# JakobHavtorn/benchmarking-lvms

Hardware: AMD Instinct MI355X
Metric: audio frames/sec training (VRNN, 16 kHz mu-law) (higher is better)
Workload: dtype f32

## Files before the change

benchmarking-lvms_amd/csrc/pchain.h:

```cpp
#pragma once
#include <algorithm>
#include <cstdlib>

#include "common.h"

namespace blvm {
namespace pchain {

constexpr unsigned SENTINEL = 0xFFFFFFFFu;
constexpr unsigned SPIN_LIMIT = 1u << 22;

typedef unsigned u32x4 __attribute__((ext_vector_type(4)));
typedef __amdgpu_buffer_rsrc_t rsrc_t;
constexpr int AUX_SC1 = 16;
#ifndef PCHAIN_POLL_AUX
#define PCHAIN_POLL_AUX AUX_SC1
#endif
#ifndef PCHAIN_STORE_AUX
#define PCHAIN_STORE_AUX AUX_SC1
#endif
__device__ __forceinline__ rsrc_t make_rsrc(const void* base) {
  const unsigned long long u = reinterpret_cast<unsigned long long>(base);
  const unsigned lo = (unsigned)__builtin_amdgcn_readfirstlane((int)(unsigned)u), hi = (unsigned)__builtin_amdgcn_readfirstlane((int)(unsigned)(u >> 32));
  return __builtin_amdgcn_make_buffer_rsrc(reinterpret_cast<void*>(((unsigned long long)hi << 32) | lo), 0, 0xFFFFFFFFu, 0x00020000);
}
__device__ __forceinline__ f32x4 ld_sc1_x4(rsrc_t r, unsigned byte_off) {
  return __builtin_bit_cast(f32x4, __builtin_amdgcn_raw_buffer_load_b128(r, (int)byte_off, 0, PCHAIN_POLL_AUX));
}
__device__ __forceinline__ float ld_sc1(rsrc_t r, unsigned byte_off) {
  return __builtin_bit_cast(float, __builtin_amdgcn_raw_buffer_load_b32(r, (int)byte_off, 0, PCHAIN_POLL_AUX));
}
__device__ __forceinline__ void st_sc1(rsrc_t r, unsigned byte_off, float v) {
  __builtin_amdgcn_raw_buffer_store_b32(__builtin_bit_cast(unsigned, v), r, (int)byte_off, 0, PCHAIN_STORE_AUX);
}

__device__ __forceinline__ bool is_sentinel(float x) { return __float_as_uint(x) == SENTINEL; }
__device__ __forceinline__ bool any_sentinel(const f32x4& v) {
  return is_sentinel(v[0]) | is_sentinel(v[1]) | is_sentinel(v[2]) | is_sentinel(v[3]);
}

struct Ctl {
  unsigned* dev;
  unsigned* host;
  unsigned epoch;
  __device__ __forceinline__ bool aborted() const { return __hip_atomic_load(dev, __ATOMIC_RELAXED, __HIP_MEMORY_SCOPE_AGENT) == epoch; }
  __device__ __forceinline__ void abort(unsigned code) const {
    if (__hip_atomic_exchange(dev, epoch, __ATOMIC_RELAXED, __HIP_MEMORY_SCOPE_AGENT) != epoch) {
      __hip_atomic_store(host + 1, code, __ATOMIC_RELAXED, __HIP_MEMORY_SCOPE_SYSTEM);
      __hip_atomic_fetch_add(host, 1u, __ATOMIC_RELAXED, __HIP_MEMORY_SCOPE_SYSTEM);
    }
  }
};

__device__ __forceinline__ bool spin_tick(unsigned& spins, const Ctl& ctl, unsigned code, bool& dead) {
  ++spins;
  if ((spins & 255u) == 0) {
    if (ctl.aborted()) { dead = true; return true; }
    if (spins >= SPIN_LIMIT) { ctl.abort(code); dead = true; return true; }
  }
  return false;
}

struct Poll {
  Ctl ctl;
  unsigned code;
  bool dead;
  int nap;
#ifdef PCHAIN_TPROF
  unsigned long long t_first = 0, t_ok = 0, t_end = 0, tp[8] = {0, 0, 0, 0, 0, 0, 0, 0};
  unsigned polls = 0;
#endif
  __device__ __forceinline__ void sleep() const {
    if (nap > 8) __builtin_amdgcn_s_sleep(32);
    else __builtin_amdgcn_s_sleep(1);
  }
};

struct MapSame { static constexpr int of(int) { return 0; } static constexpr bool sum = false; };
struct MapId { static constexpr int of(int g) { return g; } static constexpr bool sum = false; };
struct MapPairs { static constexpr int of(int g) { return g >> 1; } static constexpr bool sum = false; };
struct MapSum { static constexpr int of(int) { return 0; } static constexpr bool sum = true; };

struct NoMid {
  __device__ __forceinline__ void operator()() const {}
};

typedef short s16x4 __attribute__((ext_vector_type(4)));
typedef unsigned u32x2 __attribute__((ext_vector_type(2)));
typedef float f32x2_t __attribute__((ext_vector_type(2)));
typedef __bf16 bf16x2_t __attribute__((ext_vector_type(2)));
typedef _Float16 f16x2_t __attribute__((ext_vector_type(2)));
typedef _Float16 f16x4_t __attribute__((ext_vector_type(4)));
__device__ __forceinline__ unsigned pk_bf16(float a, float b) {
  return __builtin_bit_cast(unsigned, __builtin_convertvector((f32x2_t){a, b}, bf16x2_t));
}
template <int OT>
__device__ __forceinline__ unsigned pk16(float a, float b) {
  if constexpr (OT == OP_F16) return __builtin_bit_cast(unsigned, __builtin_convertvector((f32x2_t){a, b}, f16x2_t));
  else return pk_bf16(a, b);
}
template <int OT>
__device__ __forceinline__ f32x4 mfma16(s16x4 a, s16x4 b, f32x4 acc) {
  if constexpr (OT == OP_F16)
    return __builtin_amdgcn_mfma_f32_16x16x16f16(__builtin_bit_cast(f16x4_t, a), __builtin_bit_cast(f16x4_t, b), acc, 0, 0, 0);
  else return __builtin_amdgcn_mfma_f32_16x16x16bf16_1k(a, b, acc, 0, 0, 0);
}
template <int OT> struct WFrag { typedef u32x2 type; };
template <> struct WFrag<OP_F32> { typedef f32x4 type; };

template <int NW, int OT, int GA, int G, class AMap, int CH, class Mid>
__device__ __forceinline__ void mgemm_trip(const rsrc_t (&ar)[GA], unsigned aoff, const float* const (&ap)[GA], const char* const (&wp)[G], int kc,
                                           bool aok, bool polled, f32x4 (&acc)[G], Poll& pl, Mid& mid, bool& mid_pending) {
  constexpr int STEP = NW * 16;
  typedef typename WFrag<OT>::type wfrag;
  constexpr int ES = OT != OP_F32 ? 2 : 4;
  wfrag w[G][CH];
  f32x4 a[GA][CH];
#pragma unroll
  for (int u = 0; u < CH; ++u)
#pragma unroll
    for (int g = 0; g < G; ++g) w[g][u] = *reinterpret_cast<const wfrag*>(wp[g] + (size_t)ES * 16 * (size_t)(kc + u * STEP));
  if (!polled) {
#pragma unroll
    for (int u = 0; u < CH; ++u)
#pragma unroll
      for (int g = 0; g < GA; ++g) a[g][u] = *reinterpret_cast<const f32x4*>(ap[g] + kc + u * STEP);
    if (mid_pending) { mid(); mid_pending = false; }
  } else {
    unsigned spins = 0;
    for (;;) {
#pragma unroll
      for (int u = 0; u < CH; ++u)
#pragma unroll
        for (int g = 0; g < GA; ++g) a[g][u] = ld_sc1_x4(ar[g], aoff + 64u * (unsigned)(kc + u * STEP));
      if (mid_pending) { mid(); mid_pending = false; }
      bool bad = false;
#pragma unroll
      for (int u = 0; u < CH; ++u)
#pragma unroll
        for (int g = 0; g < GA; ++g) bad |= any_sentinel(a[g][u]);
#ifdef PCHAIN_TPROF
      if (spins == 0 && pl.t_first == 0) pl.t_first = wall_clock64();
      pl.polls++;
#endif
      if (!__any(bad && aok) || pl.dead) break;
      if (spin_tick(spins, pl.ctl, pl.code, pl.dead)) break;
      pl.sleep();
    }
#ifdef PCHAIN_TPROF
    pl.t_ok = wall_clock64();
#endif
  }
  if constexpr (AMap::sum) {
#pragma unroll
    for (int u = 0; u < CH; ++u)
#pragma unroll
      for (int ga = 1; ga < GA; ++ga) a[0][u] += a[ga][u];
  }
  if constexpr (OT != OP_F32) {
#pragma unroll
    for (int u = 0; u < CH; ++u) {
      s16x4 ab[GA];
#pragma unroll
      for (int ga = 0; ga < GA; ++ga) {
        const f32x4 x = a[ga][u];
        const u32x2 q = {aok ? pk16<OT>(x[0], x[1]) : 0u, aok ? pk16<OT>(x[2], x[3]) : 0u};
        ab[ga] = __builtin_bit_cast(s16x4, q);
      }
#pragma unroll
      for (int g = 0; g < G; ++g) acc[g] = mfma16<OT>(ab[AMap::of(g)], __builtin_bit_cast(s16x4, w[g][u]), acc[g]);
    }
  } else {
#pragma unroll
    for (int u = 0; u < CH; ++u)
#pragma unroll
      for (int e = 0; e < 4; ++e)
#pragma unroll
        for (int g = 0; g < G; ++g) acc[g] = __builtin_amdgcn_mfma_f32_16x16x4f32(aok ? a[AMap::of(g)][u][e] : 0.f, w[g][u][e], acc[g], 0, 0, 0);
  }
}

template <int NW, int OT, int GA, int G, class AMap, class Mid = NoMid>
__device__ __forceinline__ void mgemm16(const float* const (&A)[GA], const int (&lda)[GA], bool polled, int r0, int nrows,
                                        const float* const (&W)[G], const int (&c0)[G], int K, f32x4 (&acc)[G], Poll& pl, Mid mid = Mid(),
                                        int a_width = 0, int w_width = 0) {
  constexpr int STEP = NW * 16;
  constexpr int FR = (NW >= 16 ? 6 : 12) / (G + GA);
  constexpr int MAXCH = FR >= 6 ? 6 : (FR >= 4 ? 4 : (FR >= 2 ? 2 : 1));
  const int lane = threadIdx.x & 63, wave = threadIdx.x >> 6;
  const int rr = lane & 15, q = lane >> 4;
  const bool aok = (r0 + rr) < nrows;
  rsrc_t ar[GA];
  const float* ap[GA];
  const char* wp[G];
#pragma unroll
  for (int g = 0; g < GA; ++g) {
    ar[g] = make_rsrc(A[g]);
    ap[g] = A[g] + (size_t)(aok ? r0 + rr : r0) * (polled ? 0 : lda[g]) + 4 * q;
  }
  const unsigned aoff = 4u * ((unsigned)(r0 >> 4) * 16u * (unsigned)(a_width > 0 ? a_width : K) + 4u * (unsigned)lane);
#pragma unroll
  for (int g = 0; g < G; ++g) wp[g] = reinterpret_cast<const char*>(W[g]) + (OT != OP_F32 ? 2 : 4) * ((size_t)c0[g] * (w_width > 0 ? w_width : K) + 4 * lane);
  int nch = (K / 16 - wave + NW - 1) / NW;
  int kc = wave * 16;
  bool mid_pending = true;
  if constexpr (MAXCH >= 6) for (; nch >= 6; nch -= 6, kc += 6 * STEP) mgemm_trip<NW, OT, GA, G, AMap, 6>(ar, aoff, ap, wp, kc, aok, polled, acc, pl, mid, mid_pending);
  if constexpr (MAXCH >= 4) for (; nch >= 4; nch -= 4, kc += 4 * STEP) mgemm_trip<NW, OT, GA, G, AMap, 4>(ar, aoff, ap, wp, kc, aok, polled, acc, pl, mid, mid_pending);
  if constexpr (MAXCH >= 2) for (; nch >= 2; nch -= 2, kc += 2 * STEP) mgemm_trip<NW, OT, GA, G, AMap, 2>(ar, aoff, ap, wp, kc, aok, polled, acc, pl, mid, mid_pending);
  for (; nch >= 1; nch -= 1, kc += STEP) mgemm_trip<NW, OT, GA, G, AMap, 1>(ar, aoff, ap, wp, kc, aok, polled, acc, pl, mid, mid_pending);
  if (mid_pending) mid();
}

template <int N>
__device__ __forceinline__ void poll_words(const rsrc_t (&r)[N], const unsigned (&off)[N], float (&v)[N], bool need, Poll& pl) {
  unsigned spins = 0;
  for (;;) {
#pragma unroll
    for (int i = 0; i < N; ++i) v[i] = ld_sc1(r[i], off[i]);
    bool bad = false;
#pragma unroll
    for (int i = 0; i < N; ++i) bad |= is_sentinel(v[i]);
    if (!__any(bad && need) || pl.dead) break;
    if (spin_tick(spins, pl.ctl, pl.code, pl.dead)) break;
    pl.sleep();
  }
}

__device__ __forceinline__ int first_tile(int w, int wg0, int nwg, int ntiles) {
  return (w >= wg0 && w < wg0 + nwg) ? w - wg0 : ntiles;
}

struct TileIter {
  int rt, ct, j, step, x, n;
  bool xcd;
  __host__ __device__ __forceinline__ TileIter(int w, int wg0, int nwg, int rt_, int ct_, bool xcd_) : rt(rt_), ct(ct_), xcd(xcd_) {
    const int wl = w - wg0;
    const bool in = w >= wg0 && wl < nwg;
    if (xcd) {
      x = wl & 7; step = nwg >> 3; j = wl >> 3;
      n = x < ct ? ((ct - x + 7) >> 3) * rt : 0;
    } else {
      x = 0; step = nwg; j = wl;
      n = rt * ct;
    }
    if (!in || step < 1) { j = 0; n = 0; step = 1; x = 0; }
  }
  __host__ __device__ __forceinline__ bool valid() const { return j < n; }
  __host__ __device__ __forceinline__ void next() { j += step; }
  __host__ __device__ __forceinline__ int r0() const { return (j % rt) * 16; }
  __host__ __device__ __forceinline__ int c() const { return xcd ? x + 8 * (j / rt) : j / rt; }
};

inline int tiles_per_workgroup(int rt, int ct, int nwg, bool xcd) {
  if (nwg <= 0) return 0;
  if (xcd) return nwg >= 8 ? (((ct + 7) / 8) * rt + nwg / 8 - 1) / (nwg / 8) : ((ct + 7) / 8) * rt;
  return (ct * rt + nwg - 1) / nwg;
}

__device__ __forceinline__ void canary_wait(const float* A16, int r0, int K, Poll& pl, int a_width = 0) {
  if (threadIdx.x < 64) {
    const int lane = threadIdx.x, np = K >> 4;
    const rsrc_t r = make_rsrc(A16 + (size_t)(r0 >> 4) * 16 * (a_width > 0 ? a_width : K));
    unsigned spins = 0;
    for (;;) {
      bool bad = false;
      for (int p0 = 0; p0 < np; p0 += 64) {
        const int pr = p0 + lane;
        const float v = ld_sc1(r, 1024u * (unsigned)(pr < np ? pr : 0));
        bad |= (pr < np) && is_sentinel(v);
      }
      if (!__any(bad) || pl.dead) break;
      if (spin_tick(spins, pl.ctl, pl.code, pl.dead)) break;
      pl.sleep();
    }
  }
  __syncthreads();
}

struct WMem {
  static constexpr bool resident = false;
  static constexpr int products = 0;
};
template <int OT, int G, int NCH>
struct WRegs {
  static constexpr bool resident = true;
  static constexpr int products = G;
  typename WFrag<OT>::type w[G][NCH];
};
template <int NW, int OT, int G, int NCH>
__device__ __forceinline__ void load_w(typename WFrag<OT>::type (&w)[G][NCH], const float* const* W, const int (&c0)[G], int ldw) {
  typedef typename WFrag<OT>::type wfrag;
  const int lane = threadIdx.x & 63, wave = threadIdx.x >> 6;
  constexpr int ES = OT != OP_F32 ? 2 : 4;
#pragma unroll
  for (int g = 0; g < G; ++g) {
    const char* base = reinterpret_cast<const char*>(W[g]) + (size_t)ES * ((size_t)c0[g] * ldw + 4 * lane);
#pragma unroll
    for (int u = 0; u < NCH; ++u) w[g][u] = *reinterpret_cast<const wfrag*>(base + (size_t)ES * 256 * (size_t)(wave + u * NW));
  }
}
template <int NW, int OT, int GA, int G, class AMap, int NCH, bool SHARED, class Mid>
__device__ __forceinline__ void product_regs(const float* const (&A16)[GA], int r0, int nrows, int width,
                                             const typename WFrag<OT>::type (&w)[G][NCH], f32x4 (&acc)[G], Poll& pl, Mid mid) {
  static_assert(!SHARED || GA == 1, "the shared-slab form reads one operand");
  const int lane = threadIdx.x & 63, wave = threadIdx.x >> 6;
  const bool aok = (r0 + (lane & 15)) < nrows;
  rsrc_t ar[GA];
#pragma unroll
  for (int g = 0; g < GA; ++g) ar[g] = make_rsrc(A16[g]);
  const unsigned aoff = 4u * ((unsigned)(r0 >> 4) * 16u * (unsigned)width + 4u * (unsigned)lane) + 1024u * (unsigned)wave;
  f32x4 a[GA][NCH];
  unsigned spins = 0;
  bool mid_pending = true;
  if constexpr (SHARED) {
    canary_wait(A16[0], r0, width, pl);
    const float* ap = A16[0] + (size_t)(r0 >> 4) * 16 * width + 4 * lane + 256 * wave;
#pragma unroll
    for (int u = 0; u < NCH; ++u) a[0][u] = *reinterpret_cast<const f32x4*>(ap + 256 * (size_t)(u * NW));
    mid();
    mid_pending = false;
    bool bad = false;
#pragma unroll
    for (int u = 0; u < NCH; ++u) bad |= any_sentinel(a[0][u]);
    if (!__any(bad && aok)) goto multiply;
  }
  for (;;) {
#pragma unroll
    for (int u = 0; u < NCH; ++u)
#pragma unroll
      for (int g = 0; g < GA; ++g) a[g][u] = ld_sc1_x4(ar[g], aoff + 1024u * (unsigned)(u * NW));
    if (mid_pending) { mid(); mid_pending = false; }
    bool bad = false;
#pragma unroll
    for (int u = 0; u < NCH; ++u)
#pragma unroll
      for (int g = 0; g < GA; ++g) bad |= any_sentinel(a[g][u]);
    if (!__any(bad && aok) || pl.dead) break;
    if (spin_tick(spins, pl.ctl, pl.code, pl.dead)) break;
    pl.sleep();
  }
multiply:
  if constexpr (AMap::sum) {
#pragma unroll
    for (int u = 0; u < NCH; ++u)
#pragma unroll
      for (int ga = 1; ga < GA; ++ga) a[0][u] += a[ga][u];
  }
  if constexpr (OT != OP_F32) {
#pragma unroll
    for (int u = 0; u < NCH; ++u) {
      s16x4 ab[GA];
#pragma unroll
      for (int ga = 0; ga < GA; ++ga) {
        const f32x4 x = a[ga][u];
        const u32x2 q = {aok ? pk16<OT>(x[0], x[1]) : 0u, aok ? pk16<OT>(x[2], x[3]) : 0u};
        ab[ga] = __builtin_bit_cast(s16x4, q);
      }
#pragma unroll
      for (int g = 0; g < G; ++g) acc[g] = mfma16<OT>(ab[AMap::of(g)], __builtin_bit_cast(s16x4, w[g][u]), acc[g]);
    }
  } else {
#pragma unroll
    for (int u = 0; u < NCH; ++u)
#pragma unroll
      for (int e = 0; e < 4; ++e)
#pragma unroll
        for (int g = 0; g < G; ++g) acc[g] = __builtin_amdgcn_mfma_f32_16x16x4f32(aok ? a[AMap::of(g)][u][e] : 0.f, w[g][u][e], acc[g], 0, 0, 0);
  }
}

template <int NW, int OT, int GA, int G, class AMap, class Mid = NoMid>
__device__ __forceinline__ void tile_product(const WMem&, const float* const (&A)[GA], const int (&lda)[GA], bool polled, int r0, int nrows,
                                             const float* const (&W)[G], const int (&c0)[G], int K, f32x4 (&acc)[G], Poll& pl, Mid mid = Mid(),
                                             int a_width = 0, int w_width = 0) {
  mgemm16<NW, OT, GA, G, AMap>(A, lda, polled, r0, nrows, W, c0, K, acc, pl, mid, a_width, w_width);
}
template <int NW, int OT, int GA, int G, class AMap, class Mid = NoMid, int NCH>
__device__ __forceinline__ void tile_product(const WRegs<OT, G, NCH>& ws, const float* const (&A)[GA], const int (&)[GA], bool, int r0, int nrows,
                                             const float* const (&)[G], const int (&)[G], int, f32x4 (&acc)[G], Poll& pl, Mid mid = Mid(),
                                             int a_width = 0, int = 0) {
  product_regs<NW, OT, GA, G, AMap, NCH, false>(A, r0, nrows, a_width > 0 ? a_width : NCH * 16 * NW, ws.w, acc, pl, mid);
}

struct Out {
  float* rm;
  int ld;
  bool rm_sc1;
  float* x16;
  int n16;
  float* x16b = nullptr;
  int n16b = 0;
};
__device__ __forceinline__ Out out_rm(float* p, int ld, bool sc1 = false) { return Out{p, ld, sc1, nullptr, 0}; }
__device__ __forceinline__ Out out_both(float* p, int ld, float* x16, int n16, bool sc1 = false) { return Out{p, ld, sc1, x16, n16}; }
__device__ __forceinline__ void put(const Out& o, int r0, int c0, int row, int col, float x) {
  if (o.rm != nullptr) {
    if (o.rm_sc1) st_sc1(make_rsrc(o.rm), 4u * ((unsigned)row * (unsigned)o.ld + (unsigned)col), x);
    else o.rm[(size_t)row * o.ld + col] = x;
  }
  const int rr = row - r0, cc = col - c0;
  const unsigned in_block = (unsigned)((rr + 16 * ((cc & 15) >> 2)) * 4 + (cc & 3));
  if (o.x16 != nullptr) st_sc1(make_rsrc(o.x16), 4u * ((((unsigned)(r0 >> 4) * (unsigned)o.n16 + (unsigned)((c0 + cc) >> 4)) << 8) + in_block), x);
  if (o.x16b != nullptr) st_sc1(make_rsrc(o.x16b), 4u * ((((unsigned)(r0 >> 4) * (unsigned)o.n16b + (unsigned)((c0 + cc) >> 4)) << 8) + in_block), x);
}


struct LinLate {
  const float *bias, *add, *gate;
  int ldadd, ldgate;
  bool add_polled, relu;
  float slope;
  Out out;
};
template <int NW, int OT, class Late, class WS = WMem>
__device__ __forceinline__ void tile_lin_late(const float* A, int lda, bool a_polled, const float* W, int K, Late& late, int r0, int c0, int B,
                                              float* red, Poll& pl, const float* A2 = nullptr, const float* A3 = nullptr, int w_width = 0,
                                              const WS& ws = WS()) {
  const int t = threadIdx.x & 255;
  const int row = r0 + (t >> 4), col = c0 + (t & 15);
  const bool own = threadIdx.x < 256 && row < B;
  const int rowc = row < B ? row : r0;
#ifdef PCHAIN_TPROF
  const unsigned long long t0 = wall_clock64();
  pl.t_first = 0; pl.polls = 0;
#endif
  float e_bias = 0.f, e_gate = 1.f, e_add = 0.f;
  LinLate L;
  auto prefetch = [&]() {
    L = late();
    if (L.bias) e_bias = L.bias[col];
    if (L.gate) e_gate = L.gate[(size_t)rowc * L.ldgate + col];
    if (L.add && !L.add_polled) e_add = L.add[(size_t)rowc * L.ldadd + col];
  };
  f32x4 acc[1] = {{0.f, 0.f, 0.f, 0.f}};
  if (A2 != nullptr) {
    const float* const As[3] = {A, A2, A3};
    const float* const Ws[1] = {W};
    const int la[3] = {0, 0, 0}, cs[1] = {c0};
    tile_product<NW, OT, 3, 1, MapSum>(ws, As, la, true, r0, B, Ws, cs, K, acc, pl, prefetch, lda, w_width);
  } else {
    const float* const As[1] = {A};
    const float* const Ws[1] = {W};
    const int la[1] = {lda}, cs[1] = {c0};
    tile_product<NW, OT, 1, 1, MapSame>(ws, As, la, a_polled, r0, B, Ws, cs, K, acc, pl, prefetch, a_polled ? lda : 0, w_width);
  }
  float v[1];
  reduce_tiles<1, NW>(acc, red, v);
#ifdef PCHAIN_TPROF
  if (a_polled && pl.nap == 1) {
    const unsigned long long t3 = wall_clock64();
    pl.tp[0] += 1; pl.tp[1] += pl.t_first - t0; pl.tp[2] += pl.t_ok - pl.t_first; pl.tp[3] += t3 - pl.t_ok; pl.tp[4] += pl.polls;
    if (pl.t_end != 0) pl.tp[6] += t0 - pl.t_end;
  }
#endif
  if (threadIdx.x >= 256) return;
  if (L.add && L.add_polled) {
    const rsrc_t rs[1] = {make_rsrc(L.add)};
    const unsigned os[1] = {4u * ((unsigned)rowc * (unsigned)L.ldadd + (unsigned)col)};
    float ws[1];
    poll_words<1>(rs, os, ws, own, pl);
    e_add = ws[0];
  }
  if (!own) return;
  float x = v[0] + e_bias + e_add;
  if (L.relu) x = x > 0.f ? x : x * L.slope;
  if (L.gate) x = e_gate > 0.f ? x : x * L.slope;
  put(L.out, r0, c0, row, col, x);
#ifdef PCHAIN_TPROF
  if (a_polled && pl.nap == 1) { pl.t_end = wall_clock64(); }
#endif
}
template <int NW, int OT = OP_F32>
__device__ __forceinline__ void tile_lin(const float* A, int lda, bool a_polled, const float* W, int K, const float* bias,
                                         const float* add, int ldadd, bool add_polled, const float* gate, int ldgate, bool relu,
                                         float slope, const Out& out, int r0, int c0, int B, float* red, Poll& pl) {
  auto late = [&]() { return LinLate{bias, add, gate, ldadd, ldgate, add_polled, relu, slope, out}; };
  tile_lin_late<NW, OT>(A, lda, a_polled, W, K, late, r0, c0, B, red, pl);
}

struct HeadOut {
  float *mu_p, *sd_p, *mu_q, *sd_q, *raw_p, *raw_q, *muq_raw;
  Out z;
};
template <int NW, int OT = OP_F32, class WS = WMem>
__device__ __forceinline__ void tile_head(const float* P, const float* Q, bool polled, const float* Wp, const float* bp, const float* Wq,
                                          const float* bq, const float* eps, const HeadOut& o, int H, int Z, int residual, float beta,
                                          float inv_beta, float sd_eps, int r0, int c0, int B, float* red, Poll& pl, const WS& ws = WS()) {
  const int t = threadIdx.x & 255;
  const int row = r0 + (t >> 4), col = c0 + (t & 15);
  const bool own = threadIdx.x < 256 && row < B;
  const size_t oc = (size_t)(row < B ? row : r0) * Z + col;
  float b0 = 0.f, b1 = 0.f, b2 = 0.f, b3 = 0.f, e = 0.f;
  auto prefetch = [&]() { b0 = bp[col]; b1 = bp[Z + col]; b2 = bq[col]; b3 = bq[Z + col]; e = eps[oc]; };
  f32x4 acc[4];
#pragma unroll
  for (int g = 0; g < 4; ++g) acc[g] = (f32x4){0.f, 0.f, 0.f, 0.f};
  {
    const float* const As[2] = {P, Q};
    const float* const Ws[4] = {Wp, Wp, Wq, Wq};
    const int la[2] = {H, H}, cs[4] = {c0, Z + c0, c0, Z + c0};
    tile_product<NW, OT, 2, 4, MapPairs>(ws, As, la, polled, r0, B, Ws, cs, H, acc, pl, prefetch);
  }
  float v[4];
  reduce_tiles<4, NW>(acc, red, v);
  if (!own) return;
  const size_t oo = (size_t)row * Z + col;
  const float mp = v[0] + b0, rp = v[1] + b1, rq = v[3] + b3;
  float mq = v[2] + b2;
  const float sp = softplus_beta(rp, beta, inv_beta) + sd_eps;
  const float sq = softplus_beta(rq, beta, inv_beta) + sd_eps;
  if (o.muq_raw != nullptr) o.muq_raw[oo] = mq;
  float sqc = sq;
  if (residual == 1) {
    mq += mp;
  } else if (residual == 2) {
    const float pq = 1.f / (sq * sq), pp = 1.f / (sp * sp);
    const float var = 1.f / (pq + pp);
    mq = var * (mq * pq + mp * pp);
    sqc = sqrtf(var);
  } else if (residual == 3) {
    mq = mp;
    sqc = sp;
  }
  put(o.z, r0, c0, row, col, e * sqc + mq);
  o.mu_p[oo] = mp; o.sd_p[oo] = sp; o.mu_q[oo] = mq; o.sd_q[oo] = sqc;
  o.raw_p[oo] = rp; o.raw_q[oo] = rq;
}

template <int NW, int OT = OP_F32, class WS = WMem>
__device__ __forceinline__ void tile_gru(const float* X, int ldx, bool polled, const float* Wih, int K, const float* xg, const float* bih,
                                         const float* gh, const float* hprev, int ldh, int R, const Out& hnew, float* rg, float* ug, float* ng,
                                         int r0, int c0, int B, float* red, Poll& pl, const WS& ws = WS()) {
  const int t = threadIdx.x & 255;
  const int row = r0 + (t >> 4), col = c0 + (t & 15);
  const bool own = threadIdx.x < 256 && row < B;
  const int rowc = row < B ? row : r0;
  const size_t o3 = (size_t)rowc * 3 * R + col;
  const rsrc_t rgh = make_rsrc(gh), rhp = make_rsrc(hprev);
  const rsrc_t ps[4] = {rgh, rgh, rgh, rhp};
  const unsigned po[4] = {4u * (unsigned)o3, 4u * (unsigned)(o3 + R), 4u * (unsigned)(o3 + 2 * R), 4u * ((unsigned)rowc * (unsigned)ldh + (unsigned)col)};
  float w[4] = {0.f, 0.f, 0.f, 0.f}, x0 = 0.f, x1 = 0.f, x2 = 0.f;
  auto prefetch = [&]() {
#pragma unroll
    for (int i = 0; i < 4; ++i) w[i] = ld_sc1(ps[i], po[i]);
    x0 = (xg ? xg[o3] : 0.f) + (bih ? bih[col] : 0.f);
    x1 = (xg ? xg[o3 + R] : 0.f) + (bih ? bih[R + col] : 0.f);
    x2 = (xg ? xg[o3 + 2 * R] : 0.f) + (bih ? bih[2 * R + col] : 0.f);
  };
  f32x4 acc[3];
#pragma unroll
  for (int g = 0; g < 3; ++g) acc[g] = (f32x4){0.f, 0.f, 0.f, 0.f};
  {
    const float* const As[1] = {X};
    const float* const Ws[3] = {Wih, Wih, Wih};
    const int la[1] = {ldx}, cs[3] = {c0, R + c0, 2 * R + c0};
    tile_product<NW, OT, 1, 3, MapSame>(ws, As, la, polled, r0, B, Ws, cs, K, acc, pl, prefetch);
  }
  float v[3];
  reduce_tiles<3, NW>(acc, red, v);
  if (threadIdx.x >= 256) return;
  if (__any(own && (is_sentinel(w[0]) | is_sentinel(w[1]) | is_sentinel(w[2]) | is_sentinel(w[3])))) poll_words<4>(ps, po, w, own, pl);
  if (!own) return;
  const float r = sigmoidf_(v[0] + x0 + w[0]);
  const float u = sigmoidf_(v[1] + x1 + w[1]);
  const float n = tanhf(v[2] + x2 + r * w[2]);
  put(hnew, r0, c0, row, col, (1.f - u) * n + u * w[3]);
  const size_t o = (size_t)row * R + col;
  rg[o] = r; ug[o] = u; ng[o] = n;
}

struct DzIn {
  const float *mu_q, *sd_q, *mu_p, *sd_p, *eps, *raw_q, *raw_p, *muq_raw;
  const int32_t* x_sl;
  const float *c_raw, *c_fn;
  int t, stride, residual;
  float fn_floor, beta, sd_eps;
  bool has_gemm = true;
};
template <int NW, int OT = OP_F32, class WS = WMem>
__device__ __forceinline__ void tile_dz(const float* D, const float* WT, const float* D2, const float* WT2, bool polled, const float* dz_add,
                                        int ld_add, bool add_polled, const DzIn& a, const Out& dqh, const Out& dph, int H, int Z, int r0, int c0,
                                        int B, float* red, Poll& pl, const WS& ws = WS()) {
  const int t = threadIdx.x & 255;
  const int row = r0 + (t >> 4), col = c0 + (t & 15);
  const bool own = threadIdx.x < 256 && row < B;
  const int rowc = row < B ? row : r0;
  const size_t o = (size_t)rowc * Z + col;
  float mq = 0.f, sq = 1.f, mp = 0.f, sp = 1.f, e = 0.f, rq = 0.f, rp = 0.f, c_raw = 0.f, c_fn = 0.f, e_add = 0.f;
  auto prefetch = [&]() {
    mq = a.mu_q[o]; sq = a.sd_q[o]; mp = a.mu_p[o]; sp = a.sd_p[o]; e = a.eps[o]; rq = a.raw_q[o]; rp = a.raw_p[o];
    if (a.c_fn != nullptr || a.c_raw != nullptr) {
      const bool live = (long long)a.t * a.stride < a.x_sl[rowc];
      c_raw = (live && a.c_raw != nullptr) ? a.c_raw[rowc] : 0.f;
      c_fn = (live && a.c_fn != nullptr) ? a.c_fn[rowc] : 0.f;
    }
    if (dz_add != nullptr && !add_polled) e_add = dz_add[(size_t)rowc * ld_add + col];
  };
  float v[2] = {0.f, 0.f};
  if (a.has_gemm) {
    f32x4 acc[2];
    acc[0] = (f32x4){0.f, 0.f, 0.f, 0.f};
    acc[1] = (f32x4){0.f, 0.f, 0.f, 0.f};
    if (WS::products != 1 && D2 != nullptr) {
      if constexpr (WS::products != 1) {
        const float* const As[2] = {D, D2};
        const float* const Ws[2] = {WT, WT2};
        const int la[2] = {H, H}, cs[2] = {c0, c0};
        tile_product<NW, OT, 2, 2, MapId>(ws, As, la, polled, r0, B, Ws, cs, H, acc, pl, prefetch);
      }
    } else {
      if constexpr (WS::products != 2) {
        f32x4 a1[1] = {acc[0]};
        const float* const As[1] = {D};
        const float* const Ws[1] = {WT};
        const int la[1] = {H}, cs[1] = {c0};
        tile_product<NW, OT, 1, 1, MapSame>(ws, As, la, polled, r0, B, Ws, cs, H, a1, pl, prefetch);
        acc[0] = a1[0];
      }
    }
    reduce_tiles<2, NW>(acc, red, v);
  } else {
    prefetch();
  }
  if (threadIdx.x >= 256) return;
  if (dz_add != nullptr && add_polled) {
    const rsrc_t rs[1] = {make_rsrc(dz_add)};
    const unsigned os[1] = {4u * ((unsigned)rowc * (unsigned)ld_add + (unsigned)col)};
    float ws[1];
    poll_words<1>(rs, os, ws, own, pl);
    e_add = ws[0];
  }
  if (!own) return;
  const float dz = v[0] + v[1] + e_add;
  const float d = mq - mp, ip2 = 1.f / (sp * sp);
  float coef = c_raw;
  if (c_fn != 0.f) {
    const float k = logf(sp) - logf(sq) + (sq * sq + d * d) * 0.5f * ip2 - 0.5f;
    if (!(a.fn_floor > 0.f) || k > a.fn_floor) coef += c_fn;
  }
  float g_muq = dz + coef * d * ip2;
  float g_sdq = dz * e + coef * (sq * ip2 - 1.f / sq);
  float g_mup = -coef * d * ip2;
  float g_sdp = coef * (1.f / sp - (sq * sq + d * d) * ip2 / sp);
  if (a.residual == 1) {
    g_mup += g_muq;
  } else if (a.residual == 2) {
    const float mqr = a.muq_raw[o];
    const float sqr = softplus_beta(rq, a.beta, 1.f / a.beta) + a.sd_eps;
    const float pq = 1.f / (sqr * sqr), pp = ip2, var = sq * sq;
    const float half_s3 = 0.5f * var * sq;
    const float g_pq = g_muq * var * (mqr - mq) - g_sdq * half_s3;
    const float g_pp = g_muq * var * (mp - mq) - g_sdq * half_s3;
    g_mup += g_muq * var * pp;
    g_sdp += g_pp * (-2.f * pp / sp);
    g_sdq = g_pq * (-2.f * pq / sqr);
    g_muq = g_muq * var * pq;
  }
  put(dqh, r0, c0, row, col, g_muq);
  put(dqh, r0, Z + c0, row, Z + col, g_sdq * sigmoidf_(a.beta * rq));
  put(dph, r0, c0, row, col, g_mup);
  put(dph, r0, Z + c0, row, Z + col, g_sdp * sigmoidf_(a.beta * rp));
}

struct GrubIn {
  const float *D0, *D1, *W0, *W1, *g_in, *g_add;
  const float *rg, *ug, *ng, *gh, *hprev, *dd;
  int ldh, ld_gadd;
  Out dgi, dgh;
  float *ga, *g_out;
  bool has_gemm, has_gin, has_gates;
};
template <int NW, int OT = OP_F32, class WS = WMem>
__device__ __forceinline__ void tile_grub(const GrubIn& a, int K, int R, int r0, int c0, int B, float* red, Poll& pl, const WS& ws = WS()) {
  const int tt = threadIdx.x & 255;
  const int row = r0 + (tt >> 4), col = c0 + (tt & 15);
  const bool own = threadIdx.x < 256 && row < B;
  const int rowc = row < B ? row : r0;
  const size_t o = (size_t)rowc * R + col, o3 = (size_t)rowc * 3 * R + col;
  float r = 0.f, u = 0.f, n = 0.f, hn = 0.f, hp = 0.f, dd = 0.f, gadd = 0.f, g0 = 0.f;
  auto prefetch = [&]() {
    if (a.has_gin) g0 = ld_sc1(make_rsrc(a.g_in), 4u * (unsigned)o);
    if (a.has_gates) {
      r = a.rg[o]; u = a.ug[o]; n = a.ng[o]; hn = a.gh[o3 + 2 * R];
      hp = a.hprev[(size_t)rowc * a.ldh + col];
      if (a.dd != nullptr) dd = a.dd[(size_t)rowc * a.ldh + col];
    }
    if (a.g_add != nullptr) gadd = a.g_add[(size_t)rowc * a.ld_gadd + col];
  };
  float v[2] = {0.f, 0.f};
  if (!a.has_gemm) prefetch();
  if (a.has_gemm) {
    f32x4 acc[2];
    acc[0] = (f32x4){0.f, 0.f, 0.f, 0.f};
    acc[1] = (f32x4){0.f, 0.f, 0.f, 0.f};
    const float* const As[2] = {a.D0, a.D1};
    const float* const Ws[2] = {a.W0, a.W1};
    const int la[2] = {0, 0}, cs[2] = {c0, c0};
    tile_product<NW, OT, 2, 2, MapId>(ws, As, la, true, r0, B, Ws, cs, K, acc, pl, prefetch);
    reduce_tiles<2, NW>(acc, red, v);
  }
  if (threadIdx.x >= 256) return;
  if (a.has_gin && __any(own && is_sentinel(g0))) {
    const rsrc_t rs[1] = {make_rsrc(a.g_in)};
    const unsigned os[1] = {4u * (unsigned)o};
    float ws[1];
    poll_words<1>(rs, os, ws, own, pl);
    g0 = ws[0];
  }
  if (!own) return;
  const float g = (g0 + gadd) + v[0] + v[1];
  if (!a.has_gates) { a.g_out[(size_t)row * R + col] = g; return; }
  const float dn_pre = g * (1.f - u) * (1.f - n * n);
  const float du_pre = g * (hp - n) * u * (1.f - u);
  const float dr_pre = dn_pre * hn * r * (1.f - r);
  put(a.dgi, r0, c0, row, col, dr_pre); put(a.dgi, r0, R + c0, row, R + col, du_pre); put(a.dgi, r0, 2 * R + c0, row, 2 * R + col, dn_pre);
  put(a.dgh, r0, c0, row, col, dr_pre); put(a.dgh, r0, R + c0, row, R + col, du_pre); put(a.dgh, r0, 2 * R + c0, row, 2 * R + col, dn_pre * r);
  st_sc1(make_rsrc(a.ga), 4u * ((unsigned)row * (unsigned)R + (unsigned)col), g * u + dd);
}

__device__ __forceinline__ int seq_time_index(int j, int reverse, const int32_t* lens, int row) {
  if (!reverse) return j;
  const int n = lens[row];
  return j < n ? n - 1 - j : j;
}
struct GruSeqIn {
  const float *H16, *Whh, *bhh;
  const float* xg;
  const int32_t* lens;
  const float* hprev;
  float* out;
  float *rg, *ug, *ng, *ghn;
  long out_ts;
  int out_ld, j, reverse;
};
template <int NW, int OT = OP_F32>
__device__ __forceinline__ void tile_gru_seq(const GruSeqIn& a, const Out& hnext, int R, int r0, int c0, int B, float* red, Poll& pl) {
  const int t = threadIdx.x & 255;
  const int row = r0 + (t >> 4), col = c0 + (t & 15);
  const bool own = threadIdx.x < 256 && row < B;
  const int rowc = row < B ? row : r0;
  const size_t o = (size_t)rowc * R + col;
  int idx = 0;
  float x0 = 0.f, x1 = 0.f, x2 = 0.f, b0 = 0.f, b1 = 0.f, b2 = 0.f, hp = 0.f;
  auto prefetch = [&]() {
    idx = seq_time_index(a.j, a.reverse, a.lens, rowc);
    const size_t ox = ((size_t)idx * B + rowc) * 3 * R + col;
    x0 = a.xg[ox]; x1 = a.xg[ox + R]; x2 = a.xg[ox + 2 * R];
    b0 = a.bhh[col]; b1 = a.bhh[R + col]; b2 = a.bhh[2 * R + col];
    hp = a.hprev[o];
  };
  f32x4 acc[3];
#pragma unroll
  for (int g = 0; g < 3; ++g) acc[g] = (f32x4){0.f, 0.f, 0.f, 0.f};
  {
    const float* const As[1] = {a.H16};
    const float* const Ws[3] = {a.Whh, a.Whh, a.Whh};
    const int la[1] = {0}, cs[3] = {c0, R + c0, 2 * R + c0};
    mgemm16<NW, OT, 1, 3, MapSame>(As, la, true, r0, B, Ws, cs, R, acc, pl, prefetch);
  }
  float v[3];
  reduce_tiles<3, NW>(acc, red, v);
  if (!own) return;
  const float hn = v[2] + b2;
  const float r = sigmoidf_(x0 + v[0] + b0);
  const float u = sigmoidf_(x1 + v[1] + b1);
  const float n = tanhf(x2 + r * hn);
  const float h2 = (1.f - u) * n + u * hp;
  put(hnext, r0, c0, row, col, h2);
  a.out[(size_t)idx * a.out_ts + (size_t)row * a.out_ld + col] = h2;
  a.rg[o] = r; a.ug[o] = u; a.ng[o] = n; a.ghn[o] = hn;
}

struct GruSeqBwdIn {
  const float *DGHn16, *WhhT;
  const float* dout;
  const float *rg, *ug, *ng, *ghn, *hprev;
  const int32_t* lens;
  float* G;
  float* DGI;
  float* dh0;
  long out_ts;
  int out_ld, j, reverse;
  bool has_gemm, has_gates;
};
template <int NW, int OT = OP_F32>
__device__ __forceinline__ void tile_gru_seq_bwd(const GruSeqBwdIn& a, const Out& dgh, int R, int r0, int c0, int B, float* red, Poll& pl) {
  const int t = threadIdx.x & 255;
  const int row = r0 + (t >> 4), col = c0 + (t & 15);
  const bool own = threadIdx.x < 256 && row < B;
  const int rowc = row < B ? row : r0;
  const size_t o = (size_t)rowc * R + col;
  float g = 0.f, dout = 0.f, r = 0.f, u = 0.f, n = 0.f, hn = 0.f, hp = 0.f;
  int idx = 0;
  auto prefetch = [&]() {
    g = a.G[o];
    if (a.has_gates) {
      idx = seq_time_index(a.j, a.reverse, a.lens, rowc);
      dout = a.dout[(size_t)idx * a.out_ts + (size_t)rowc * a.out_ld + col];
      r = a.rg[o]; u = a.ug[o]; n = a.ng[o]; hn = a.ghn[o]; hp = a.hprev[o];
    }
  };
  float v[1] = {0.f};
  if (a.has_gemm) {
    f32x4 acc[1] = {{0.f, 0.f, 0.f, 0.f}};
    const float* const As[1] = {a.DGHn16};
    const float* const Ws[1] = {a.WhhT};
    const int la[1] = {0}, cs[1] = {c0};
    mgemm16<NW, OT, 1, 1, MapSame>(As, la, true, r0, B, Ws, cs, 3 * R, acc, pl, prefetch);
    reduce_tiles<1, NW>(acc, red, v);
  } else {
    prefetch();
    __syncthreads();
  }
  if (!own) return;
  g += dout + v[0];
  if (!a.has_gates) { a.dh0[o] = g; return; }
  const float dn_pre = g * (1.f - u) * (1.f - n * n);
  const float du_pre = g * (hp - n) * u * (1.f - u);
  const float dr_pre = dn_pre * hn * r * (1.f - r);
  const size_t oi = ((size_t)idx * B + row) * 3 * R + col;
  a.DGI[oi] = dr_pre; a.DGI[oi + R] = du_pre; a.DGI[oi + 2 * R] = dn_pre;
  put(dgh, r0, c0, row, col, dr_pre);
  put(dgh, r0, R + c0, row, R + col, du_pre);
  put(dgh, r0, 2 * R + c0, row, 2 * R + col, dn_pre * r);
  a.G[o] = g * u;
}

struct LstmSeqIn {
  const float *H16, *Whh, *bhh;
  const float* xg;
  const int32_t* lens;
  const float *hprev, *cprev;
  float *cnext, *out, *gates;
  int t;
};
template <int NW, int OT = OP_F32>
__device__ __forceinline__ void tile_lstm_seq(const LstmSeqIn& a, const Out& hnext, int H, int r0, int c0, int B, float* red, Poll& pl) {
  const int tt = threadIdx.x & 255;
  const int row = r0 + (tt >> 4), col = c0 + (tt & 15);
  const bool own = threadIdx.x < 256 && row < B;
  const int rowc = row < B ? row : r0;
  const size_t o = (size_t)rowc * H + col, o4 = (size_t)rowc * 4 * H + col;
  float x0 = 0.f, x1 = 0.f, x2 = 0.f, x3 = 0.f, hp = 0.f, cp = 0.f;
  bool live = true;
  auto prefetch = [&]() {
    x0 = a.xg[o4] + a.bhh[col]; x1 = a.xg[o4 + H] + a.bhh[H + col];
    x2 = a.xg[o4 + 2 * H] + a.bhh[2 * H + col]; x3 = a.xg[o4 + 3 * H] + a.bhh[3 * H + col];
    hp = a.hprev[o]; cp = a.cprev[o];
    live = a.lens == nullptr || a.t < a.lens[rowc];
  };
  f32x4 acc[4];
#pragma unroll
  for (int g = 0; g < 4; ++g) acc[g] = (f32x4){0.f, 0.f, 0.f, 0.f};
  {
    const float* const As[1] = {a.H16};
    const float* const Ws[4] = {a.Whh, a.Whh, a.Whh, a.Whh};
    const int la[1] = {0}, cs[4] = {c0, H + c0, 2 * H + c0, 3 * H + c0};
    mgemm16<NW, OT, 1, 4, MapSame>(As, la, true, r0, B, Ws, cs, H, acc, pl, prefetch);
  }
  float v[4];
  reduce_tiles<4, NW>(acc, red, v);
  if (!own) return;
  const float i = sigmoidf_(v[0] + x0), f = sigmoidf_(v[1] + x1), g = tanhf(v[2] + x2), og = sigmoidf_(v[3] + x3);
  const float c2 = f * cp + i * g;
  const float h2 = og * tanhf(c2);
  a.cnext[o] = live ? c2 : cp;
  put(hnext, r0, c0, row, col, live ? h2 : hp);
  a.out[o] = live ? h2 : 0.f;
  a.gates[o4] = live ? i : 0.f;
  a.gates[o4 + H] = live ? f : 0.f;
  a.gates[o4 + 2 * H] = live ? g : 0.f;
  a.gates[o4 + 3 * H] = live ? og : 0.f;
}

struct LstmSeqBwdIn {
  const float *DGn16, *WhhT;
  const float *dout, *gates, *c_s, *c_s1;
  float* DC;
  float* dh0;
  bool has_gemm, has_gates;
};
template <int NW, int OT = OP_F32>
__device__ __forceinline__ void tile_lstm_seq_bwd(const LstmSeqBwdIn& a, const Out& dg, int H, int r0, int c0, int B, float* red, Poll& pl) {
  const int tt = threadIdx.x & 255;
  const int row = r0 + (tt >> 4), col = c0 + (tt & 15);
  const bool own = threadIdx.x < 256 && row < B;
  const int rowc = row < B ? row : r0;
  const size_t o = (size_t)rowc * H + col, o4 = (size_t)rowc * 4 * H + col;
  float dh = 0.f, ig = 0.f, fg = 0.f, gg = 0.f, og = 0.f, cs = 0.f, cs1 = 0.f, dc = 0.f;
  auto prefetch = [&]() {
    if (a.has_gates) {
      dh = a.dout[o];
      ig = a.gates[o4]; fg = a.gates[o4 + H]; gg = a.gates[o4 + 2 * H]; og = a.gates[o4 + 3 * H];
      cs = a.c_s[o]; cs1 = a.c_s1[o]; dc = a.DC[o];
    }
  };
  float v[1] = {0.f};
  if (a.has_gemm) {
    f32x4 acc[1] = {{0.f, 0.f, 0.f, 0.f}};
    const float* const As[1] = {a.DGn16};
    const float* const Ws[1] = {a.WhhT};
    const int la[1] = {0}, cs_[1] = {c0};
    mgemm16<NW, OT, 1, 1, MapSame>(As, la, true, r0, B, Ws, cs_, 4 * H, acc, pl, prefetch);
    reduce_tiles<1, NW>(acc, red, v);
  } else {
    prefetch();
    __syncthreads();
  }
  if (!own) return;
  dh += v[0];
  if (!a.has_gates) { a.dh0[o] = dh; return; }
  const float tc = tanhf(cs1);
  const float d_o = dh * tc;
  const float dct = dc + dh * og * (1.f - tc * tc);
  put(dg, r0, c0, row, col, dct * gg * ig * (1.f - ig));
  put(dg, r0, H + c0, row, H + col, dct * cs * fg * (1.f - fg));
  put(dg, r0, 2 * H + c0, row, 2 * H + col, dct * ig * (1.f - gg * gg));
  put(dg, r0, 3 * H + c0, row, 3 * H + col, d_o * og * (1.f - og));
  a.DC[o] = dct * fg;
}

template <int NW, int OT = OP_F32>
__device__ __forceinline__ void tile_lstm(const float* X, const float* Wih, int K, const float* bih, const float* gh, const float* cprev, float* cnext, int H,
                                          const Out& hnew, int r0, int c0, int B, float* red, Poll& pl) {
  const int t = threadIdx.x & 255;
  const int row = r0 + (t >> 4), col = c0 + (t & 15);
  const bool own = threadIdx.x < 256 && row < B;
  const int rowc = row < B ? row : r0;
  const size_t o = (size_t)rowc * H + col, o4 = (size_t)rowc * 4 * H + col;
  const rsrc_t rgh = make_rsrc(gh);
  const rsrc_t ps[4] = {rgh, rgh, rgh, rgh};
  const unsigned po[4] = {4u * (unsigned)o4, 4u * (unsigned)(o4 + H), 4u * (unsigned)(o4 + 2 * H), 4u * (unsigned)(o4 + 3 * H)};
  float w[4] = {0.f, 0.f, 0.f, 0.f}, b0 = 0.f, b1 = 0.f, b2 = 0.f, b3 = 0.f, cp = 0.f;
  auto prefetch = [&]() {
#pragma unroll
    for (int i = 0; i < 4; ++i) w[i] = ld_sc1(ps[i], po[i]);
    b0 = bih[col]; b1 = bih[H + col]; b2 = bih[2 * H + col]; b3 = bih[3 * H + col];
    cp = cprev[o];
  };
  f32x4 acc[4];
#pragma unroll
  for (int g = 0; g < 4; ++g) acc[g] = (f32x4){0.f, 0.f, 0.f, 0.f};
  {
    const float* const As[1] = {X};
    const float* const Ws[4] = {Wih, Wih, Wih, Wih};
    const int la[1] = {0}, cs[4] = {c0, H + c0, 2 * H + c0, 3 * H + c0};
    mgemm16<NW, OT, 1, 4, MapSame>(As, la, true, r0, B, Ws, cs, K, acc, pl, prefetch);
  }
  float v[4];
  reduce_tiles<4, NW>(acc, red, v);
  if (threadIdx.x >= 256) return;
  if (__any(own && (is_sentinel(w[0]) | is_sentinel(w[1]) | is_sentinel(w[2]) | is_sentinel(w[3])))) poll_words<4>(ps, po, w, own, pl);
  if (!own) return;
  const float i = sigmoidf_(v[0] + b0 + w[0]), f = sigmoidf_(v[1] + b1 + w[1]), g = tanhf(v[2] + b2 + w[2]), og = sigmoidf_(v[3] + b3 + w[3]);
  const float c2 = f * cp + i * g;
  cnext[(size_t)row * H + col] = c2;
  put(hnew, r0, c0, row, col, og * tanhf(c2));
}

template <int NW>
__device__ __forceinline__ void tile_dmol_sample(const float* dec, int ldd, const float* Wl, const float* bl, const float* u, const float* v, int S, int F,
                                                 int num_mix, float log_eps, const Out& xo, int r0, int s0, int B, float* lds, Poll& pl) {
  static_assert(NW == 8 || NW == 16, "waves");
  const int tid = threadIdx.x, wave = tid >> 6, lane = tid & 63;
  float* in = lds;
  float* outp = lds + 16 * 4 * F;
  const int rowlen = 4 * F;
  const int pieces = 16 * rowlen / 4;
  const rsrc_t rd = make_rsrc(dec);
  {
    unsigned spins = 0;
    for (;;) {
      bool bad = false;
      for (int q = tid; q < pieces; q += NW * 64) {
        const int rr = q / (rowlen / 4), cq = q % (rowlen / 4);
        const bool ok = r0 + rr < B;
        const f32x4 x = ld_sc1_x4(rd, 4u * ((unsigned)(ok ? r0 + rr : r0) * (unsigned)ldd + (unsigned)(s0 * F + 4 * cq)));
        bad |= ok && any_sentinel(x);
        *reinterpret_cast<f32x4*>(in + rr * rowlen + 4 * cq) = x;
      }
      if (!__any(bad) || pl.dead) break;
      if (spin_tick(spins, pl.ctl, pl.code, pl.dead)) break;
      pl.sleep();
    }
  }
  __syncthreads();
  {
    const int rr = lane >> 2, ss = lane & 3;
    const float* a = in + rr * rowlen + ss * F;
    if (wave * 4 < F) {
      float acc[4];
#pragma unroll
      for (int j = 0; j < 4; ++j) {
        const int jj = wave * 4 + j;
        acc[j] = jj < F ? bl[jj] : 0.f;
      }
      for (int k = 0; k < F; ++k) {
        const float ak = a[k];
#pragma unroll
        for (int j = 0; j < 4; ++j) {
          const int jj = wave * 4 + j;
          if (jj < F) acc[j] = fmaf(Wl[jj * F + k], ak, acc[j]);
        }
      }
#pragma unroll
      for (int j = 0; j < 4; ++j)
        if (wave * 4 + j < F) outp[lane * 32 + wave * 4 + j] = acc[j];
    }
  }
  __syncthreads();
  if (wave == 0) {
    const int rr = lane >> 2, ss = lane & 3, row = r0 + rr, smp = s0 + ss;
    if (row < B) {
      const float* p = outp + lane * 32;
      const size_t f = (size_t)row * S + smp;
      int best = 0;
      float bv = -INFINITY;
      for (int m = 0; m < num_mix; ++m) {
        float sc = p[m];
        if (u != nullptr) sc -= logf(-logf(u[f * num_mix + m]));
        if (sc > bv) { bv = sc; best = m; }
      }
      const float loc = p[num_mix + best], raw = p[2 * num_mix + best];
      float x = loc;
      if (v != nullptr) {
        const float vv = v[f];
        x = loc + expf(fmaxf(raw, log_eps)) * (logf(vv) - logf(1.f - vv));
        x = fminf(fmaxf(x, -1.f), 1.f);
      }
      put(xo, r0, s0 & ~15, row, smp, x);
    }
  }
  __syncthreads();
}

enum Kind : int { K_LIN = 0, K_HEAD = 1, K_GRU = 2, K_DZ = 3, K_GRUB = 4, K_DMOLS = 5, K_GRUS = 6, K_GRUSB = 7, K_LSTMS = 8, K_LSTMSB = 9, K_LINSEQ = 10, K_LSTM = 11 };
enum DescFlag : int {
  DF_RELU = 1,
  DF_A_PLAIN = 2,
  DF_ADD_POLLED = 4,
  DF_RM_SC1 = 8,
  DF_GENTLE = 16,
  DF_CANARY = 32,
  DF_A_SUM3 = 64,
  DF_SEQ_GATE = 128,
};
enum : int { LD_OUT = 3, N16_OUT = 0, N16_OUTB = 1 };
enum : int { LIN_A, LIN_W, LIN_BIAS, LIN_ADD, LIN_GATE, LIN_ORM, LIN_O16, LIN_O16B, LIN_A2, LIN_A3, LIN_LD_A = 0, LIN_LD_ADD = 1, LIN_LD_GATE = 2,
             LIN_I_W_WIDTH = 0, LIN_F_SLOPE = 0 };
enum : int { LINSEQ_A0 = 0, LINSEQ_W = 1, LINSEQ_AUX = 5, LINSEQ_ORM = 9, LINSEQ_O16 = 13, LINSEQ_ADD0 = 17, LINSEQ_LD_ORM = 0,
             LINSEQ_I_LD_ADD0 = 0, LINSEQ_I_N = 1, LINSEQ_I_LD_GATE = 2, LINSEQ_I_K0 = 3, LINSEQ_F_SLOPE = 0 };
enum : int { HEAD_P16, HEAD_Q16, HEAD_WP, HEAD_BP, HEAD_WQ, HEAD_BQ, HEAD_EPS, HEAD_MU_P, HEAD_SD_P, HEAD_MU_Q, HEAD_SD_Q, HEAD_RAW_P, HEAD_RAW_Q,
             HEAD_MUQ_RAW, HEAD_Z, HEAD_Z16, HEAD_Z16B, HEAD_I_Z = 0, HEAD_I_RESIDUAL = 1, HEAD_F_BETA = 0, HEAD_F_INV_BETA = 1, HEAD_F_SD_EPS = 2 };
enum : int { GRU_X16, GRU_WIH, GRU_XG, GRU_GH, GRU_HPREV, GRU_HRM, GRU_H16, GRU_RG, GRU_UG, GRU_NG, GRU_BIH, GRU_H16B, GRU_LD_HPREV = 0, GRU_I_R = 0 };
enum : int { DZ_D16, DZ_WT, DZ_D2_16, DZ_WT2, DZ_ADD, DZ_MU_Q, DZ_SD_Q, DZ_MU_P, DZ_SD_P, DZ_EPS, DZ_RAW_Q, DZ_RAW_P, DZ_MUQ_RAW, DZ_X_SL, DZ_C_RAW,
             DZ_C_FN, DZ_DQH, DZ_DQH16, DZ_DPH, DZ_DPH16, DZ_LD_ADD = 1, DZ_I_Z = 0, DZ_I_RESIDUAL = 1, DZ_I_STRIDE = 2, DZ_I_T0 = 3,
             DZ_F_FN_FLOOR = 0, DZ_F_BETA = 1, DZ_F_SD_EPS = 2, DZ_F_GEMM_FROM = 3 };
enum : int { GRUB_D0_16, GRUB_D1_16, GRUB_W0, GRUB_W1, GRUB_G_IN, GRUB_RG, GRUB_UG, GRUB_NG, GRUB_GH, GRUB_HPREV, GRUB_DD, GRUB_DGI, GRUB_DGI16,
             GRUB_DGH, GRUB_DGH16, GRUB_GA, GRUB_G_OUT, GRUB_G_ADD, GRUB_LD_H = 0, GRUB_LD_GADD = 1, GRUB_I_R = 0, GRUB_I_GEMM_FROM = 1,
             GRUB_I_GATES_TO = 2, GRUB_I_GIN_FROM = 3 };
enum : int { DMOLS_DEC, DMOLS_W, DMOLS_B, DMOLS_U, DMOLS_V, DMOLS_X, DMOLS_X16, DMOLS_LD_DEC = 0, DMOLS_I_S = 0, DMOLS_I_F = 1, DMOLS_I_NMIX = 2,
             DMOLS_F_LOG_EPS = 0 };
enum : int { GRUS_H16, GRUS_WHH, GRUS_BHH, GRUS_XG, GRUS_LENS, GRUS_HPREV, GRUS_HNEXT, GRUS_HNEXT16, GRUS_OUT, GRUS_RG, GRUS_UG, GRUS_NG, GRUS_GHN,
             GRUS_I_R = 0, GRUS_I_REVERSE = 1, GRUS_I_OUT_TS = 2, GRUS_I_OUT_LD = 3 };
enum : int { GRUSB_DGH16_IN, GRUSB_WHHT, GRUSB_DOUT, GRUSB_RG, GRUSB_UG, GRUSB_NG, GRUSB_GHN, GRUSB_HPREV, GRUSB_LENS, GRUSB_G, GRUSB_DGI, GRUSB_DGH,
             GRUSB_DGH16, GRUSB_DH0, GRUSB_N16_T = 1, GRUSB_I_R = 0, GRUSB_I_REVERSE = 1, GRUSB_I_OUT_TS = 2, GRUSB_I_OUT_LD = 3 };
enum : int { LSTMS_H16, LSTMS_WHH, LSTMS_BHH, LSTMS_XG, LSTMS_LENS, LSTMS_HPREV, LSTMS_HNEXT, LSTMS_HNEXT16, LSTMS_CPREV, LSTMS_CNEXT, LSTMS_OUT,
             LSTMS_GATES, LSTMS_I_H = 0 };
enum : int { LSTMSB_DG16_IN, LSTMSB_WHHT, LSTMSB_DOUT, LSTMSB_GATES, LSTMSB_CS, LSTMSB_DC, LSTMSB_DG, LSTMSB_DG16, LSTMSB_DH0, LSTMSB_N16_T = 1, LSTMSB_I_H = 0 };
enum : int { LSTM_X16, LSTM_WIH, LSTM_BIH, LSTM_GH, LSTM_CPREV, LSTM_CNEXT, LSTM_HRM, LSTM_H16, LSTM_H16B, LSTM_I_H = 0 };
constexpr int kMaxDesc = 24, kMaxPtr = 20;
struct Desc {
  int kind, ct, wg0, nwg, flags, K, s_begin, s_end;
  int ld[4];
  int n16[2];
  int i[4];
  float f[4];
  unsigned char sidx[kMaxPtr];
  const float* p[kMaxPtr];
};
struct Program {
  int ot = OP_F32;
  int rt_group = 1;
  int s_first = 0;
  int ndesc, S, B, xcd;
  long stride[16];
  Ctl ctl;
  unsigned long long* prof;
  int prof_wg, lds_products;
  Desc d[kMaxDesc];
};

struct Ptr {
  const void* p; long step;
  Ptr(const void* p_ = nullptr, long step_ = 0) : p(p_), step(step_) {}
};
struct Builder {
  Program p{};
  int nstride = 1;
  bool overflow = false;
  void begin(int ot, int S, int B, int lds_products, bool backward, int prof_wg) {
    p.ot = ot; p.S = S; p.B = B; p.xcd = (pchain_tune() & 4) ? 1 : 0; p.lds_products = lds_products;
    p.prof = pchain_profile_buffer() && backward ? pchain_profile_buffer() + 64 : pchain_profile_buffer(); p.prof_wg = prof_wg;
  }
  int stride_index(long v) {
    if (v == 0) return 0;
    for (int i = 1; i < nstride; ++i)
      if (p.stride[i] == v) return i;
    if (nstride >= 16) { overflow = true; return 0; }
    p.stride[nstride] = v;
    return nstride++;
  }
  Desc& add(int kind, int ct, int wg0, int nwg, int K, int flags, int s_begin, int s_end) {
    static Desc dummy;
    if (p.ndesc >= kMaxDesc) { overflow = true; return dummy; }
    Desc& d = p.d[p.ndesc++];
    d = Desc{};
    d.kind = kind; d.ct = ct; d.wg0 = wg0; d.nwg = nwg; d.K = K; d.flags = flags; d.s_begin = s_begin; d.s_end = s_end;
    return d;
  }
  void ptr(Desc& d, int k, Ptr q) {
    d.p[k] = static_cast<const float*>(q.p);
    d.sidx[k] = (unsigned char)(q.p ? stride_index(q.step) : 0);
  }
};
inline Ptr rev(const float* base, long step, long t0) { return Ptr(base ? base + t0 * step : nullptr, -step); }

struct Operands {
  Ptr p[kMaxPtr];
  int ld[4] = {}, n16[2] = {}, i[4] = {}; float f[4] = {};
};
inline Desc& add_desc(Builder& b, int kind, int ct, int wg0, int nwg, int K, int flags, int s_begin, int s_end, const Operands& o) {
  Desc& d = b.add(kind, ct, wg0, nwg, K, flags, s_begin, s_end);
  for (int k = 0; k < kMaxPtr; ++k) b.ptr(d, k, o.p[k]);
  std::copy(o.ld, o.ld + 4, d.ld); std::copy(o.n16, o.n16 + 2, d.n16); std::copy(o.i, o.i + 4, d.i); std::copy(o.f, o.f + 4, d.f);
  return d;
}

struct SeqLink {
  const float *W, *aux;
  float* orm;
  long rm_step;
  int ldo;
  float* o16;
};
inline Desc& add_linseq(Builder& b, int ct, int wg0, int nwg, int K, bool relu, bool gated, int s_begin, int s_end, Ptr A16, int n, const SeqLink* L,
                        long aux_step, long o16_step, int n16, float slope, int ldgate, int K0 = 0, Ptr add0 = Ptr(), int ldadd0 = 0) {
  Desc& d = b.add(K_LINSEQ, ct, wg0, nwg, K, (relu ? DF_RELU : 0) | (gated ? DF_SEQ_GATE : 0), s_begin, s_end);
  b.ptr(d, LINSEQ_A0, A16); b.ptr(d, LINSEQ_ADD0, add0);
  d.i[LINSEQ_I_K0] = (K0 != 0 && K0 != K) ? K0 : 0; d.i[LINSEQ_I_LD_ADD0] = ldadd0;
  for (int i = 0; i < n && i < 4; ++i) {
    b.ptr(d, LINSEQ_W + i, L[i].W); b.ptr(d, LINSEQ_AUX + i, Ptr(L[i].aux, gated ? aux_step : 0)); b.ptr(d, LINSEQ_ORM + i, Ptr(L[i].orm, L[i].rm_step));
    b.ptr(d, LINSEQ_O16 + i, Ptr(L[i].o16, o16_step)); d.ld[LINSEQ_LD_ORM + i] = L[i].ldo;
  }
  if (n > 4) b.overflow = true;
  d.n16[N16_OUT] = n16; d.i[LINSEQ_I_N] = n; d.i[LINSEQ_I_LD_GATE] = ldgate; d.f[LINSEQ_F_SLOPE] = slope;
  return d;
}
inline SeqLink rev_link(const float* W, const float* gate, float* orm, float* o16, long t0, long sB, int ld, long x16) {
  return SeqLink{W, gate ? gate + t0 * sB : nullptr, orm ? orm + t0 * sB : nullptr, -sB, ld, o16 ? o16 + t0 * x16 : nullptr};
}
inline int range_for(int tiles, int avail) { return std::max(8, std::min(avail & ~7, (tiles + 7) & ~7)); }

}

hipError_t pchain_fill_sentinel(void* p, size_t bytes, hipStream_t stream);
inline int pchain_ctl(pchain::Ctl& c) { return pchain_ctl(&c.dev, &c.host, &c.epoch); }
int pchain_prepare(pchain::Builder& bld, const char* who);
int pchain_run(const pchain::Program& prog, hipStream_t stream);
inline int pchain_launch(pchain::Builder& bld, const char* who, hipStream_t stream) {
  BLVM_TRY(pchain_prepare(bld, who));
  return pchain_run(bld.p, stream);
}
int vrnn_launch(pchain::Builder& bld, bool forward, const char* who, hipStream_t stream);
int pchain_rows_to_t16(const float* src, int ld, int B, int K, float* dst, hipStream_t stream, int n16 = 0);
inline int device_cus() {
  static int v = [] {
    int dev = 0, n = 0;
    if (hipGetDevice(&dev) != hipSuccess) return 0;
    if (hipDeviceGetAttribute(&n, hipDeviceAttributeMultiprocessorCount, dev) != hipSuccess) return 0;
    if (const char* e = getenv("BLVM_PCHAIN_CUS")) {
      const int m = atoi(e) & ~7;
      if (m >= 32 && m < n) n = m;
    }
    return n;
  }();
  return v;
}
constexpr int kPchainCarveMaxB = 128;
inline bool pchain_applies(int B) { return B <= pchain_max_batch() && B <= kPchainCarveMaxB; }
inline OpType pchain_optype(int B) { return operand_16bit() && pchain_applies(B) && device_cus() >= 32 ? operand_type() : OP_F32; }

}
```

benchmarking-lvms_amd/csrc/vrnn_static.hip:

```cpp
#include <algorithm>
#include <mutex>

#include "common.h"
#include "pchain.h"
#include "vrnn_static.h"

namespace blvm {
namespace {
using namespace pchain;

struct SPtr {
  float* base;
  int stride;
  __device__ __forceinline__ float* at(int s) const { return base + (long)s * stride; }
};

constexpr int kMaxTiles = 8;
__device__ __forceinline__ int tile_lanes(int w, int wg0, int nwg, int rt, int ct, bool xcd) {
  TileIter it(w, wg0, nwg, rt, ct, xcd);
  const int lane = threadIdx.x & 63;
  it.j += lane * it.step;
  return (lane < kMaxTiles && it.valid()) ? (it.r0() | (it.c() << 16)) : -1;
}
__device__ __forceinline__ int tile_count(int lanes) { return __popcll(__ballot(lanes >= 0)); }

struct LinChainArgs {
  SPtr a16, orm, o16;
  const float *W, *bias;
  int ldo, n16, B, s0, S, wg0, nwg, ct, xcd;
  Ctl ctl;
};

template <int NW, int K, bool RES>
__global__ __launch_bounds__(NW * 64, 1) void static_lin_chain_kernel(LinChainArgs a) {
  __shared__ __attribute__((aligned(16))) float red[2][NW * 256];
  const int w = blockIdx.x, B = a.B;
  const int tiles = tile_lanes(w, a.wg0, a.nwg, (B + 15) / 16, a.ct, a.xcd != 0);
  const int nt = tile_count(tiles);
  if (nt == 0) return;
  Poll pl{a.ctl, 0u, false, 1};
  int par = 0;
  if constexpr (RES) {
    const int trc = __builtin_amdgcn_readlane(tiles, 0), r0 = trc & 0xffff, c0 = (trc >> 16) * 16;
    WRegs<OP_F32, 1, K / (16 * NW)> ws;
    const float* const Ws[1] = {a.W};
    const int cs[1] = {c0};
    load_w<NW, OP_F32, 1, K / (16 * NW)>(ws.w, Ws, cs, K);
    for (int s = a.s0; s < a.S; ++s) {
      pl.code = (unsigned)s << 4;
      auto late = [&]() { return LinLate{a.bias, nullptr, nullptr, 0, 0, false, true, 0.f, Out{a.orm.at(s), a.ldo, false, a.o16.at(s), a.n16}}; };
      tile_lin_late<NW, OP_F32>(a.a16.at(s), 0, true, a.W, K, late, r0, c0, B, red[par], pl, nullptr, nullptr, 0, ws);
      par ^= 1;
    }
    return;
  }
  for (int s = a.s0; s < a.S; ++s) {
    pl.code = (unsigned)s << 4;
    const float* A = a.a16.at(s);
    auto late = [&]() { return LinLate{a.bias, nullptr, nullptr, 0, 0, false, true, 0.f, Out{a.orm.at(s), a.ldo, false, a.o16.at(s), a.n16}}; };
    for (int tk = 0; tk < nt; ++tk) {
      const int trc = __builtin_amdgcn_readlane(tiles, tk);
      tile_lin_late<NW, false>(A, 0, true, a.W, K, late, trc & 0xffff, (trc >> 16) * 16, B, red[par], pl);
      par ^= 1;
    }
  }
}

constexpr int kH = 256, kR = 512;

struct LinArgs {
  SPtr a, a2, a3, add, gate, orm, o16, o16b;
  const float *W, *bias;
  int ld0, ld1, ld2, ld3, n16, n16b, w_width;
  float slope;
};
struct SeqArgs {
  SPtr a0, add0, aux[4], orm[4], o16[4];
  const float* W[4];
  int ld[4], ldadd0, ldgate, n16;
  float slope;
};
struct HeadArgs {
  SPtr P, Q, eps, mu_p, sd_p, mu_q, sd_q, raw_p, raw_q, muq_raw, z, z16, z16b;
  const float *Wp, *bp, *Wq, *bq;
  int ld3, n16, n16b, Z, residual;
  float beta, inv_beta, sd_eps;
};
struct GruArgs {
  SPtr X, xg, gh, hprev, hrm, h16, h16b, rg, ug, ng;
  const float *Wih, *bih;
  int ld0, ld3, n16, n16b, R;
};
struct DzArgs {
  SPtr D, add, mu_q, sd_q, mu_p, sd_p, eps, raw_q, raw_p, muq_raw, dqh, dqh16, dph, dph16;
  const float *WT, *c_raw, *c_fn;
  const int32_t* x_sl;
  int ld1, ld3, n16, Z, residual, stride, t0, first_gemm;
  float fn_floor, beta, sd_eps;
};
struct GrubArgs {
  SPtr D0, D1, g_in, rg, ug, ng, gh, hprev, dd, dgi, dgi16, dgh, dgh16, ga, g_add;
  const float *W0, *W1, *g_out;
  int ld0, ld1, ld3, n16, R, first_gemm, end_gates, first_gin;
};
struct Deal {
  int wg0, nwg, ct, s_begin, s_end, idx;
};

struct Walk {
  float* red0;
  float* red1;
  int par, B;
  Poll pl;
  __device__ __forceinline__ float* red() { par ^= 1; return par ? red0 : red1; }
  __device__ __forceinline__ void at(const Deal& d, int s, bool gentle, unsigned li = 0) {
    pl.nap = gentle ? 16 : 1;
    pl.code = ((unsigned)s << 4) | (unsigned)d.idx | (li << 28);
  }
};

template <int K, int G = 1>
using Res = WRegs<OP_F32, G, K / 256>;
template <int N, int K0, int K>
struct RunRes {
  Res<K0> first;
  Res<K> rest[N - 1];
};
__device__ __forceinline__ int tile_c0(int tiles) { return (__builtin_amdgcn_readlane(tiles, 0) >> 16) * 16; }

template <int NW, int K>
__device__ __forceinline__ void load_lin(Res<K>& r, const float* W, int ldw, int tiles, int nt) {
  if (nt == 0) return;
  const float* const Ws[1] = {W};
  const int cs[1] = {tile_c0(tiles)};
  load_w<NW, OP_F32, 1, K / 256>(r.w, Ws, cs, ldw > 0 ? ldw : K);
}
template <int NW, int N, int K0, int K>
__device__ __forceinline__ void load_run(RunRes<N, K0, K>& r, const SeqArgs& q, int tiles, int nt) {
  load_lin<NW, K0>(r.first, q.W[0], K0, tiles, nt);
#pragma unroll
  for (int li = 1; li < N; ++li) load_lin<NW, K>(r.rest[li - 1], q.W[li], K, tiles, nt);
}
template <int NW>
__device__ __forceinline__ void load_head(Res<kH, 4>& r, const HeadArgs& q, int tiles, int nt) {
  if (nt == 0) return;
  const int c0 = tile_c0(tiles);
  const float* const Ws[4] = {q.Wp, q.Wp, q.Wq, q.Wq};
  const int cs[4] = {c0, q.Z + c0, c0, q.Z + c0};
  load_w<NW, OP_F32, 4, 1>(r.w, Ws, cs, kH);
}
template <int NW>
__device__ __forceinline__ void load_gru(Res<kH, 3>& r, const GruArgs& q, int tiles, int nt) {
  if (nt == 0) return;
  const int c0 = tile_c0(tiles);
  const float* const Ws[3] = {q.Wih, q.Wih, q.Wih};
  const int cs[3] = {c0, q.R + c0, 2 * q.R + c0};
  load_w<NW, OP_F32, 3, 1>(r.w, Ws, cs, kH);
}
template <int NW>
__device__ __forceinline__ void load_grub(Res<kH, 2>& r, const GrubArgs& q, int tiles, int nt) {
  if (nt == 0) return;
  const int c0 = tile_c0(tiles);
  const float* const Ws[2] = {q.W0, q.W1};
  const int cs[2] = {c0, c0};
  load_w<NW, OP_F32, 2, 1>(r.w, Ws, cs, kH);
}

template <int NW, int K, int FLAGS, class WS>
__device__ __forceinline__ void visit_lin(const LinArgs& q, const Deal& d, int s, int tiles, int nt, Walk& wk, const WS& ws) {
  if (nt == 0 || s < d.s_begin || s >= d.s_end) return;
  constexpr bool sum3 = (FLAGS & DF_A_SUM3) != 0;
  wk.at(d, s, (FLAGS & DF_GENTLE) != 0);
  const float* A = q.a.at(s);
  const float* A2 = sum3 ? q.a2.at(s) : nullptr;
  const float* A3 = sum3 ? q.a3.at(s) : nullptr;
  auto late = [&]() {
    return LinLate{q.bias, q.add.at(s), q.gate.at(s), q.ld1, q.ld2, (FLAGS & DF_ADD_POLLED) != 0, (FLAGS & DF_RELU) != 0, q.slope,
                   Out{q.orm.at(s), q.ld3, (FLAGS & DF_RM_SC1) != 0, q.o16.at(s), q.n16, q.o16b.at(s), q.n16b}};
  };
  for (int tk = 0; tk < (WS::resident ? 1 : nt); ++tk) {
    const int trc = __builtin_amdgcn_readlane(tiles, tk), tr0 = trc & 0xffff, tc0 = (trc >> 16) * 16;
    if constexpr ((FLAGS & DF_CANARY) != 0) canary_wait(A, tr0, K, wk.pl, q.ld0);
    tile_lin_late<NW, OP_F32>(A, q.ld0, true, q.W, K, late, tr0, tc0, wk.B, wk.red(), wk.pl, A2, A3, q.w_width, ws);
  }
}

template <int NW, int N, int K0, int K, bool GATED>
__device__ __forceinline__ void visit_run(const SeqArgs& q, const Deal& d, int s, int tiles, int nt, Walk& wk, const RunRes<N, K0, K>& rr) {
  if (nt == 0 || s < d.s_begin || s >= d.s_end) return;
  const int trc = __builtin_amdgcn_readlane(tiles, 0), tr0 = trc & 0xffff, tc0 = (trc >> 16) * 16;
  const float* A = q.a0.at(s);
#pragma unroll
  for (int li = 0; li < N; ++li) {
    wk.at(d, s, false, (unsigned)li);
    auto late = [&]() {
      const float* aux = q.aux[li].at(s);
      return LinLate{GATED ? nullptr : aux, li == 0 ? q.add0.at(s) : nullptr, GATED ? aux : nullptr, q.ldadd0, q.ldgate, false, !GATED, q.slope,
                     Out{q.orm[li].at(s), q.ld[li], false, q.o16[li].at(s), q.n16}};
    };
    if (li == 0) tile_lin_late<NW, OP_F32>(A, 0, true, q.W[li], K0, late, tr0, tc0, wk.B, wk.red(), wk.pl, nullptr, nullptr, 0, rr.first);
    else tile_lin_late<NW, OP_F32>(A, 0, true, q.W[li], K, late, tr0, tc0, wk.B, wk.red(), wk.pl, nullptr, nullptr, 0, rr.rest[li > 0 ? li - 1 : 0]);
    A = q.o16[li].at(s);
  }
}

template <int NW>
__device__ __forceinline__ void visit_head(const HeadArgs& q, const Deal& d, int s, int tiles, int nt, Walk& wk, const Res<kH, 4>& ws) {
  if (nt == 0 || s < d.s_begin || s >= d.s_end) return;
  wk.at(d, s, false);
  const HeadOut o{q.mu_p.at(s), q.sd_p.at(s), q.mu_q.at(s), q.sd_q.at(s), q.raw_p.at(s), q.raw_q.at(s), q.muq_raw.at(s),
                  Out{q.z.at(s), q.ld3, false, q.z16.at(s), q.n16, q.z16b.at(s), q.n16b}};
  const int trc = __builtin_amdgcn_readlane(tiles, 0);
  tile_head<NW, OP_F32>(q.P.at(s), q.Q.at(s), true, q.Wp, q.bp, q.Wq, q.bq, q.eps.at(s), o, kH, q.Z, q.residual, q.beta, q.inv_beta, q.sd_eps,
                        trc & 0xffff, (trc >> 16) * 16, wk.B, wk.red(), wk.pl, ws);
}

template <int NW>
__device__ __forceinline__ void visit_gru(const GruArgs& q, const Deal& d, int s, int tiles, int nt, Walk& wk, const Res<kH, 3>& ws) {
  if (nt == 0 || s < d.s_begin || s >= d.s_end) return;
  wk.at(d, s, false);
  const Out o{q.hrm.at(s), q.ld3, true, q.h16.at(s), q.n16, q.h16b.at(s), q.n16b};
  const int trc = __builtin_amdgcn_readlane(tiles, 0);
  tile_gru<NW, OP_F32>(q.X.at(s), 0, true, q.Wih, kH, q.xg.at(s), q.bih, q.gh.at(s), q.hprev.at(s), q.ld0, q.R, o, q.rg.at(s), q.ug.at(s), q.ng.at(s),
                       trc & 0xffff, (trc >> 16) * 16, wk.B, wk.red(), wk.pl, ws);
}

template <int NW>
__device__ __forceinline__ void visit_dz(const DzArgs& q, const Deal& d, int s, int tiles, int nt, Walk& wk, const Res<kH>& ws) {
  if (nt == 0 || s < d.s_begin || s >= d.s_end) return;
  wk.at(d, s, false);
  DzIn z;
  z.mu_q = q.mu_q.at(s); z.sd_q = q.sd_q.at(s); z.mu_p = q.mu_p.at(s); z.sd_p = q.sd_p.at(s); z.eps = q.eps.at(s); z.raw_q = q.raw_q.at(s);
  z.raw_p = q.raw_p.at(s); z.muq_raw = q.muq_raw.at(s);
  z.x_sl = q.x_sl; z.c_raw = q.c_raw; z.c_fn = q.c_fn;
  z.t = q.t0 - s; z.stride = q.stride; z.residual = q.residual;
  z.fn_floor = q.fn_floor; z.beta = q.beta; z.sd_eps = q.sd_eps;
  z.has_gemm = s >= q.first_gemm;
  const Out oq{q.dqh.at(s), q.ld3, false, q.dqh16.at(s), q.n16}, op{q.dph.at(s), q.ld3, false, q.dph16.at(s), q.n16};
  const int trc = __builtin_amdgcn_readlane(tiles, 0);
  tile_dz<NW, OP_F32>(q.D.at(s), q.WT, nullptr, nullptr, true, q.add.at(s), q.ld1, false, z, oq, op, kH, q.Z, trc & 0xffff, (trc >> 16) * 16, wk.B,
                      wk.red(), wk.pl, ws);
}

template <int NW>
__device__ __forceinline__ void visit_grub(const GrubArgs& q, const Deal& d, int s, int tiles, int nt, Walk& wk, const Res<kH, 2>& ws) {
  if (nt == 0 || s < d.s_begin || s >= d.s_end) return;
  wk.at(d, s, false);
  GrubIn g;
  g.D0 = q.D0.at(s); g.D1 = q.D1.at(s); g.W0 = q.W0; g.W1 = q.W1; g.g_in = q.g_in.at(s); g.g_add = q.g_add.at(s); g.ld_gadd = q.ld1;
  g.rg = q.rg.at(s); g.ug = q.ug.at(s); g.ng = q.ng.at(s); g.gh = q.gh.at(s); g.hprev = q.hprev.at(s); g.dd = q.dd.at(s); g.ldh = q.ld0;
  g.dgi = Out{q.dgi.at(s), q.ld3, false, q.dgi16.at(s), q.n16};
  g.dgh = Out{q.dgh.at(s), q.ld3, false, q.dgh16.at(s), q.n16};
  g.ga = q.ga.at(s); g.g_out = const_cast<float*>(q.g_out);
  g.has_gemm = s >= q.first_gemm; g.has_gates = s < q.end_gates; g.has_gin = s >= q.first_gin;
  const int trc = __builtin_amdgcn_readlane(tiles, 0);
  tile_grub<NW, OP_F32>(g, kH, q.R, trc & 0xffff, (trc >> 16) * 16, wk.B, wk.red(), wk.pl, ws);
}

template <class A>
__device__ __forceinline__ const A& kargs() {
  typedef const __attribute__((address_space(4))) char kchar;
  kchar* p = (kchar*)__builtin_amdgcn_kernarg_segment_ptr();
  asm volatile("" : "+s"(p));
  return *(const A*)p;
}

struct FwdArgs {
  LinArgs hproj;
  SeqArgs run[2];
  HeadArgs head;
  SeqArgs phi;
  GruArgs gru;
  Deal deal[6];
  int B, s0, S, xcd;
  Ctl ctl;
};
constexpr int kFwdProducts = 4, kBwdProducts = 2;

template <int NW, int HALF>
__device__ __forceinline__ void fwd_half(const FwdArgs& a, int w, int rt, bool xcd, Walk& wk) {
  const int t1 = tile_lanes(w, a.deal[1 + HALF].wg0, a.deal[1 + HALF].nwg, rt, a.deal[1 + HALF].ct, xcd), n1 = tile_count(t1);
  const int t3 = tile_lanes(w, a.deal[3].wg0, a.deal[3].nwg, rt, a.deal[3].ct, xcd), n3 = tile_count(t3);
  const int t4 = tile_lanes(w, a.deal[4].wg0, a.deal[4].nwg, rt, a.deal[4].ct, xcd), n4 = tile_count(t4);
  const int t5 = tile_lanes(w, a.deal[5].wg0, a.deal[5].nwg, rt, a.deal[5].ct, xcd), n5 = tile_count(t5);
  RunRes<3, kR, kH> run;
  Res<kH, 4> head;
  RunRes<4, kH, kH> phi;
  Res<kH, 3> gru;
  load_run<NW>(run, kargs<FwdArgs>().run[HALF], t1, n1);
  load_head<NW>(head, kargs<FwdArgs>().head, t3, n3);
  load_run<NW>(phi, kargs<FwdArgs>().phi, t4, n4);
  load_gru<NW>(gru, kargs<FwdArgs>().gru, t5, n5);
  for (int s = a.s0; s < a.S; ++s) {
    visit_run<NW, 3, kR, kH, false>(kargs<FwdArgs>().run[HALF], kargs<FwdArgs>().deal[1 + HALF], s, t1, n1, wk, run);
    visit_head<NW>(kargs<FwdArgs>().head, kargs<FwdArgs>().deal[3], s, t3, n3, wk, head);
    visit_run<NW, 4, kH, kH, false>(kargs<FwdArgs>().phi, kargs<FwdArgs>().deal[4], s, t4, n4, wk, phi);
    visit_gru<NW>(kargs<FwdArgs>().gru, kargs<FwdArgs>().deal[5], s, t5, n5, wk, gru);
  }
}

template <int NW>
__global__ __launch_bounds__(NW * 64, 1) void vrnn_static_fwd_kernel(FwdArgs a) {
  extern __shared__ __attribute__((aligned(16))) float lds_red[];
  const int w = blockIdx.x, rt = (a.B + 15) / 16;
  const bool xcd = a.xcd != 0;
  Walk wk{lds_red, lds_red + kFwdProducts * NW * 256, 0, a.B, Poll{a.ctl, 0u, false, 1}};
  if (w >= a.deal[0].wg0) {
    const int t0 = tile_lanes(w, a.deal[0].wg0, a.deal[0].nwg, rt, a.deal[0].ct, xcd), n0 = tile_count(t0);
    if (n0 == 0) return;
    for (int s = a.s0; s < a.S; ++s) visit_lin<NW, kR, DF_RM_SC1 | DF_GENTLE | DF_CANARY>(kargs<FwdArgs>().hproj, kargs<FwdArgs>().deal[0], s, t0, n0, wk, WMem());
    return;
  }
  if (w < a.deal[2].wg0) fwd_half<NW, 0>(a, w, rt, xcd, wk);
  else fwd_half<NW, 1>(a, w, rt, xcd, wk);
}

struct BwdArgs {
  GrubArgs grub;
  LinArgs part[3], gb, sum;
  SeqArgs phi;
  DzArgs dz;
  SeqArgs run[2];
  Deal deal[10];
  int B, s0, S, xcd;
  Ctl ctl;
};

template <int NW, int HALF>
__device__ __forceinline__ void bwd_half(const BwdArgs& a, int w, int rt, bool xcd, Walk& wk) {
  const int t0 = tile_lanes(w, a.deal[0].wg0, a.deal[0].nwg, rt, a.deal[0].ct, xcd), n0 = tile_count(t0);
  const int t1 = tile_lanes(w, a.deal[1 + HALF].wg0, a.deal[1 + HALF].nwg, rt, a.deal[1 + HALF].ct, xcd), n1 = tile_count(t1);
  const int t5 = tile_lanes(w, a.deal[5].wg0, a.deal[5].nwg, rt, a.deal[5].ct, xcd), n5 = tile_count(t5);
  const int t6 = tile_lanes(w, a.deal[6].wg0, a.deal[6].nwg, rt, a.deal[6].ct, xcd), n6 = tile_count(t6);
  const int t7 = tile_lanes(w, a.deal[7].wg0, a.deal[7].nwg, rt, a.deal[7].ct, xcd), n7 = tile_count(t7);
  const int t8 = tile_lanes(w, a.deal[8 + HALF].wg0, a.deal[8 + HALF].nwg, rt, a.deal[8 + HALF].ct, xcd), n8 = tile_count(t8);
  Res<kH, 2> grub;
  Res<kR> part;
  Res<kH> sum, dz;
  RunRes<2, kH, kH> phi;
  RunRes<3, 2 * kH, kH> run;
  load_grub<NW>(grub, kargs<BwdArgs>().grub, t0, n0);
  load_lin<NW, kR>(part, kargs<BwdArgs>().part[HALF].W, kargs<BwdArgs>().part[HALF].w_width, t1, n1);
  load_lin<NW, kH>(sum, kargs<BwdArgs>().sum.W, kH, t5, n5);
  load_run<NW>(phi, kargs<BwdArgs>().phi, t6, n6);
  load_lin<NW, kH>(dz, kargs<BwdArgs>().dz.WT, kH, t7, n7);
  load_run<NW>(run, kargs<BwdArgs>().run[HALF], t8, n8);
  for (int s = a.s0; s < a.S; ++s) {
    visit_grub<NW>(kargs<BwdArgs>().grub, kargs<BwdArgs>().deal[0], s, t0, n0, wk, grub);
    visit_lin<NW, kR, 0>(kargs<BwdArgs>().part[HALF], kargs<BwdArgs>().deal[1 + HALF], s, t1, n1, wk, part);
    visit_lin<NW, kH, DF_A_SUM3>(kargs<BwdArgs>().sum, kargs<BwdArgs>().deal[5], s, t5, n5, wk, sum);
    visit_run<NW, 2, kH, kH, true>(kargs<BwdArgs>().phi, kargs<BwdArgs>().deal[6], s, t6, n6, wk, phi);
    visit_dz<NW>(kargs<BwdArgs>().dz, kargs<BwdArgs>().deal[7], s, t7, n7, wk, dz);
    visit_run<NW, 3, 2 * kH, kH, true>(kargs<BwdArgs>().run[HALF], kargs<BwdArgs>().deal[8 + HALF], s, t8, n8, wk, run);
  }
}

template <int NW>
__global__ __launch_bounds__(NW * 64, 1) void vrnn_static_bwd_kernel(BwdArgs a) {
  extern __shared__ __attribute__((aligned(16))) float lds_red[];
  const int w = blockIdx.x, rt = (a.B + 15) / 16;
  const bool xcd = a.xcd != 0;
  Walk wk{lds_red, lds_red + kBwdProducts * NW * 256, 0, a.B, Poll{a.ctl, 0u, false, 1}};
  if (w >= a.deal[3].wg0) {
    const int t = tile_lanes(w, a.deal[3].wg0, a.deal[3].nwg, rt, a.deal[3].ct, xcd), n = tile_count(t);
    if (n == 0) return;
    Res<kR> part;
    load_lin<NW, kR>(part, kargs<BwdArgs>().part[2].W, kargs<BwdArgs>().part[2].w_width, t, n);
    for (int s = a.s0; s < a.S; ++s) visit_lin<NW, kR, 0>(kargs<BwdArgs>().part[2], kargs<BwdArgs>().deal[3], s, t, n, wk, part);
    return;
  }
  if (w >= a.deal[4].wg0) {
    const int t = tile_lanes(w, a.deal[4].wg0, a.deal[4].nwg, rt, a.deal[4].ct, xcd), n = tile_count(t);
    if (n == 0) return;
    for (int s = a.s0; s < a.S; ++s)
      visit_lin<NW, 3 * kR, DF_ADD_POLLED | DF_RM_SC1 | DF_GENTLE | DF_CANARY>(kargs<BwdArgs>().gb, kargs<BwdArgs>().deal[4], s, t, n, wk, WMem());
    return;
  }
  if (w < a.deal[2].wg0) bwd_half<NW, 0>(a, w, rt, xcd, wk);
  else bwd_half<NW, 1>(a, w, rt, xcd, wk);
}

bool int_strides(const Program& p) {
  for (long v : p.stride)
    if (v < -2147483647L || v > 2147483647L) return false;
  return true;
}
SPtr sptr(const Program& p, const Desc& d, int k) { return SPtr{const_cast<float*>(d.p[k]), (int)p.stride[d.sidx[k]]}; }

template <class Kern>
int static_go(Kern kernel, int slot, int grid, size_t lds, const char* what) {
  static std::mutex mu;
  static int attr_dev[3] = {-1, -1, -1}, occ[3] = {0, 0, 0};
  int dev = 0, cus = 0;
  BLVM_HIP(hipGetDevice(&dev));
  BLVM_HIP(hipDeviceGetAttribute(&cus, hipDeviceAttributeMultiprocessorCount, dev));
  {
    std::lock_guard<std::mutex> lock(mu);
    if (attr_dev[slot] != dev) {
      BLVM_HIP(hipFuncSetAttribute(reinterpret_cast<const void*>(kernel), hipFuncAttributeMaxDynamicSharedMemorySize, (int)lds));
      BLVM_HIP(hipOccupancyMaxActiveBlocksPerMultiprocessor(&occ[slot], kernel, 1024, lds));
      attr_dev[slot] = dev;
    }
    BLVM_REQUIRE((long)occ[slot] * cus >= grid, "%s: %d workgroups are not co-resident (%d per CU x %d CUs)", what, grid, occ[slot], cus);
  }
  return BLVM_OK;
}

int static_lin_chain_launch(const Program& p, hipStream_t stream, bool resident) {
  if (p.ndesc != 1 || p.ot != OP_F32 || p.rt_group != 1 || !int_strides(p)) return 1;
  const Desc& d = p.d[0];
  if (d.kind != K_LIN || d.flags != DF_RELU || d.f[LIN_F_SLOPE] != 0.f || (d.K != 256 && d.K != 512) || d.s_begin != 0 || d.s_end != p.S) return 1;
  if (d.ld[LIN_LD_A] != 0 || d.i[LIN_I_W_WIDTH] != 0 || d.p[LIN_ADD] || d.p[LIN_GATE] || d.p[LIN_O16B] || d.p[LIN_A2] || d.p[LIN_A3] || d.n16[N16_OUTB] != 0)
    return 1;
  const int rt = (p.B + 15) / 16;
  if (d.nwg <= 0 || (p.xcd && d.nwg % 8 != 0) || tiles_per_workgroup(rt, d.ct, d.nwg, p.xcd != 0) > (resident ? 1 : kMaxTiles)) return 1;
  LinChainArgs a{sptr(p, d, LIN_A), sptr(p, d, LIN_ORM), sptr(p, d, LIN_O16), d.p[LIN_W], d.p[LIN_BIAS], d.ld[LD_OUT], d.n16[N16_OUT], p.B, p.s_first, p.S,
                 d.wg0, d.nwg, d.ct, p.xcd, p.ctl};
  const int grid = d.wg0 + d.nwg;
  auto go = [&](auto kernel) -> int {
    BLVM_TRY(static_go(kernel, 2, grid, 0, "static_lin_chain"));
    hipLaunchKernelGGL(kernel, dim3(grid), dim3(1024), 0, stream, a);
    BLVM_CHECK_LAUNCH("static_lin_chain");
    return BLVM_OK;
  };
  if (resident) return d.K == 256 ? go(&static_lin_chain_kernel<16, 256, true>) : go(&static_lin_chain_kernel<16, 512, true>);
  return d.K == 256 ? go(&static_lin_chain_kernel<16, 256, false>) : go(&static_lin_chain_kernel<16, 512, false>);
}

int g_static = 1;
long g_static_launches = 0;
bool pchain_static_on() { return g_static != 0; }

SPtr sp(const Program& p, const Desc& d, int k) { return SPtr{const_cast<float*>(d.p[k]), d.p[k] ? (int)p.stride[d.sidx[k]] : 0}; }
Deal deal_of(const Desc& d, int idx) { return Deal{d.wg0, d.nwg, d.ct, d.s_begin, d.s_end, idx}; }
bool within(const Desc& d, int lo, int hi) { return d.wg0 >= lo && d.wg0 + d.nwg <= hi; }
bool few_tiles(const Program& p, const Desc& d) {
  if (d.nwg <= 0 || (p.xcd && d.nwg % 8 != 0)) return false;
  return tiles_per_workgroup((p.B + 15) / 16, d.ct, d.nwg, p.xcd != 0) <= kMaxTiles;
}
bool shaped(const Desc& d, int kind, int flags, int K) { return d.kind == kind && d.flags == flags && d.K == K; }
bool run(const Desc& d, int n, int K0) { return d.i[LINSEQ_I_N] == n && d.i[LINSEQ_I_K0] == K0; }

LinArgs lin_args(const Program& p, const Desc& d) {
  return LinArgs{sp(p, d, LIN_A), sp(p, d, LIN_A2), sp(p, d, LIN_A3), sp(p, d, LIN_ADD), sp(p, d, LIN_GATE), sp(p, d, LIN_ORM), sp(p, d, LIN_O16),
                 sp(p, d, LIN_O16B), d.p[LIN_W], d.p[LIN_BIAS], d.ld[LIN_LD_A], d.ld[LIN_LD_ADD], d.ld[LIN_LD_GATE], d.ld[LD_OUT], d.n16[N16_OUT], d.n16[N16_OUTB],
                 d.i[LIN_I_W_WIDTH], d.f[LIN_F_SLOPE]};
}
SeqArgs seq_args(const Program& p, const Desc& d) {
  SeqArgs q{};
  q.a0 = sp(p, d, LINSEQ_A0); q.add0 = sp(p, d, LINSEQ_ADD0);
  for (int i = 0; i < d.i[LINSEQ_I_N]; ++i) {
    q.W[i] = d.p[LINSEQ_W + i]; q.aux[i] = sp(p, d, LINSEQ_AUX + i); q.orm[i] = sp(p, d, LINSEQ_ORM + i); q.o16[i] = sp(p, d, LINSEQ_O16 + i);
    q.ld[i] = d.ld[LINSEQ_LD_ORM + i];
  }
  q.ldadd0 = d.i[LINSEQ_I_LD_ADD0]; q.ldgate = d.i[LINSEQ_I_LD_GATE]; q.n16 = d.n16[N16_OUT]; q.slope = d.f[LINSEQ_F_SLOPE];
  return q;
}

int vrnn_static_check(const Program& p, int ndesc, int products) {
  if (!pchain_static_on() || p.ndesc != ndesc || p.ot != OP_F32 || p.rt_group != 1 || p.s_first != 0 || p.B > 64) return 1;
  if (p.lds_products != products || !int_strides(p)) return 1;
  for (int i = 0; i < p.ndesc; ++i)
    if (!few_tiles(p, p.d[i])) return 1;
  return 0;
}

int vrnn_static_fwd(const Program& p, hipStream_t stream) {
  if (vrnn_static_check(p, 6, kFwdProducts)) return 1;
  const Desc* d = p.d;
  const int S = p.S;
  for (int i = 0; i < 6; ++i)
    if (d[i].s_begin != 0 || d[i].s_end != S) return 1;
  if (!shaped(d[0], K_LIN, DF_RM_SC1 | DF_GENTLE | DF_CANARY, kR) || !shaped(d[1], K_LINSEQ, DF_RELU, kH) || !shaped(d[2], K_LINSEQ, DF_RELU, kH) ||
      !shaped(d[3], K_HEAD, 0, kH) || !shaped(d[4], K_LINSEQ, DF_RELU, kH) || !shaped(d[5], K_GRU, 0, kH))
    return 1;
  if (!run(d[1], 3, kR) || !run(d[2], 3, kR) || !run(d[4], 4, 0)) return 1;
  if (!one_tile_each(p, kFwdResident)) return 1;
  const int half = d[2].wg0, gentle = d[0].wg0;
  if (d[1].wg0 != 0 || !within(d[1], 0, half) || !within(d[2], half, gentle) || d[0].nwg <= 0) return 1;
  for (int i = 3; i < 6; ++i)
    if (!within(d[i], 0, gentle)) return 1;
  FwdArgs a{};
  a.hproj = lin_args(p, d[0]);
  a.run[0] = seq_args(p, d[1]); a.run[1] = seq_args(p, d[2]); a.phi = seq_args(p, d[4]);
  const Desc &h = d[3], &g = d[5];
  a.head = HeadArgs{sp(p, h, HEAD_P16), sp(p, h, HEAD_Q16), sp(p, h, HEAD_EPS), sp(p, h, HEAD_MU_P), sp(p, h, HEAD_SD_P), sp(p, h, HEAD_MU_Q),
                    sp(p, h, HEAD_SD_Q), sp(p, h, HEAD_RAW_P), sp(p, h, HEAD_RAW_Q), sp(p, h, HEAD_MUQ_RAW), sp(p, h, HEAD_Z), sp(p, h, HEAD_Z16),
                    sp(p, h, HEAD_Z16B), h.p[HEAD_WP], h.p[HEAD_BP], h.p[HEAD_WQ], h.p[HEAD_BQ], h.ld[LD_OUT], h.n16[N16_OUT], h.n16[N16_OUTB],
                    h.i[HEAD_I_Z], h.i[HEAD_I_RESIDUAL], h.f[HEAD_F_BETA], h.f[HEAD_F_INV_BETA], h.f[HEAD_F_SD_EPS]};
  a.gru = GruArgs{sp(p, g, GRU_X16), sp(p, g, GRU_XG), sp(p, g, GRU_GH), sp(p, g, GRU_HPREV), sp(p, g, GRU_HRM), sp(p, g, GRU_H16), sp(p, g, GRU_H16B),
                  sp(p, g, GRU_RG), sp(p, g, GRU_UG), sp(p, g, GRU_NG), g.p[GRU_WIH], g.p[GRU_BIH], g.ld[GRU_LD_HPREV], g.ld[LD_OUT], g.n16[N16_OUT],
                  g.n16[N16_OUTB], g.i[GRU_I_R]};
  int grid = 0;
  for (int i = 0; i < 6; ++i) { a.deal[i] = deal_of(d[i], i); grid = std::max(grid, d[i].wg0 + d[i].nwg); }
  a.B = p.B; a.s0 = p.s_first; a.S = S; a.xcd = p.xcd; a.ctl = p.ctl;
  const size_t lds = sizeof(float) * 2 * kFwdProducts * 16 * 256;
  BLVM_TRY(static_go(&vrnn_static_fwd_kernel<16>, 0, grid, lds, "vrnn_static_fwd"));
  hipLaunchKernelGGL(vrnn_static_fwd_kernel<16>, dim3(grid), dim3(1024), lds, stream, a);
  BLVM_CHECK_LAUNCH("vrnn_static_fwd");
  ++g_static_launches;
  return BLVM_OK;
}

int vrnn_static_bwd(const Program& p, hipStream_t stream) {
  if (vrnn_static_check(p, 10, kBwdProducts)) return 1;
  const Desc* d = p.d;
  const int S = p.S;
  for (int i = 0; i < 10; ++i)
    if (d[i].s_begin != 0 || d[i].s_end != (i == 0 ? S : S - 1)) return 1;
  if (!shaped(d[0], K_GRUB, 0, kH) || !shaped(d[1], K_LIN, 0, kR) || !shaped(d[2], K_LIN, 0, kR) || !shaped(d[3], K_LIN, 0, kR) ||
      !shaped(d[4], K_LIN, DF_ADD_POLLED | DF_RM_SC1 | DF_GENTLE | DF_CANARY, 3 * kR) || !shaped(d[5], K_LIN, DF_A_SUM3, kH) ||
      !shaped(d[6], K_LINSEQ, DF_SEQ_GATE, kH) || !shaped(d[7], K_DZ, 0, kH) || !shaped(d[8], K_LINSEQ, DF_SEQ_GATE, kH) ||
      !shaped(d[9], K_LINSEQ, DF_SEQ_GATE, kH))
    return 1;
  if (!run(d[6], 2, 0) || !run(d[8], 3, 2 * kH) || !run(d[9], 3, 2 * kH)) return 1;
  if (!one_tile_each(p, kBwdResident) || d[7].p[DZ_D2_16] != nullptr) return 1;
  const int half = d[2].wg0, gentle = d[4].wg0, spare = d[3].wg0;
  if (!within(d[1], 0, half) || !within(d[8], 0, half) || !within(d[2], half, gentle) || !within(d[9], half, gentle) || !within(d[4], gentle, spare) ||
      d[3].nwg <= 0)
    return 1;
  for (int i : {0, 5, 6, 7})
    if (!within(d[i], 0, gentle)) return 1;
  BwdArgs a{};
  const Desc& g = d[0];
  a.grub = GrubArgs{sp(p, g, GRUB_D0_16), sp(p, g, GRUB_D1_16), sp(p, g, GRUB_G_IN), sp(p, g, GRUB_RG), sp(p, g, GRUB_UG), sp(p, g, GRUB_NG), sp(p, g, GRUB_GH),
                    sp(p, g, GRUB_HPREV), sp(p, g, GRUB_DD), sp(p, g, GRUB_DGI), sp(p, g, GRUB_DGI16), sp(p, g, GRUB_DGH), sp(p, g, GRUB_DGH16), sp(p, g, GRUB_GA),
                    sp(p, g, GRUB_G_ADD), g.p[GRUB_W0], g.p[GRUB_W1], g.p[GRUB_G_OUT], g.ld[GRUB_LD_H], g.ld[GRUB_LD_GADD], g.ld[LD_OUT], g.n16[N16_OUT],
                    g.i[GRUB_I_R], g.i[GRUB_I_GEMM_FROM], g.i[GRUB_I_GATES_TO], g.i[GRUB_I_GIN_FROM]};
  for (int k = 0; k < 3; ++k) a.part[k] = lin_args(p, d[1 + k]);
  a.gb = lin_args(p, d[4]); a.sum = lin_args(p, d[5]);
  a.phi = seq_args(p, d[6]); a.run[0] = seq_args(p, d[8]); a.run[1] = seq_args(p, d[9]);
  const Desc& z = d[7];
  a.dz = DzArgs{sp(p, z, DZ_D16), sp(p, z, DZ_ADD), sp(p, z, DZ_MU_Q), sp(p, z, DZ_SD_Q), sp(p, z, DZ_MU_P), sp(p, z, DZ_SD_P),
                sp(p, z, DZ_EPS), sp(p, z, DZ_RAW_Q), sp(p, z, DZ_RAW_P), sp(p, z, DZ_MUQ_RAW), sp(p, z, DZ_DQH), sp(p, z, DZ_DQH16), sp(p, z, DZ_DPH),
                sp(p, z, DZ_DPH16), z.p[DZ_WT], z.p[DZ_C_RAW], z.p[DZ_C_FN], reinterpret_cast<const int32_t*>(z.p[DZ_X_SL]), z.ld[DZ_LD_ADD],
                z.ld[LD_OUT], z.n16[N16_OUT], z.i[DZ_I_Z], z.i[DZ_I_RESIDUAL], z.i[DZ_I_STRIDE], z.i[DZ_I_T0], (int)z.f[DZ_F_GEMM_FROM], z.f[DZ_F_FN_FLOOR],
                z.f[DZ_F_BETA], z.f[DZ_F_SD_EPS]};
  int grid = 0;
  for (int i = 0; i < 10; ++i) { a.deal[i] = deal_of(d[i], i); grid = std::max(grid, d[i].wg0 + d[i].nwg); }
  a.B = p.B; a.s0 = p.s_first; a.S = S; a.xcd = p.xcd; a.ctl = p.ctl;
  const size_t lds = sizeof(float) * 2 * kBwdProducts * 16 * 256;
  BLVM_TRY(static_go(&vrnn_static_bwd_kernel<16>, 1, grid, lds, "vrnn_static_bwd"));
  hipLaunchKernelGGL(vrnn_static_bwd_kernel<16>, dim3(grid), dim3(1024), lds, stream, a);
  BLVM_CHECK_LAUNCH("vrnn_static_bwd");
  ++g_static_launches;
  return BLVM_OK;
}

}

int vrnn_launch(pchain::Builder& bld, bool forward, const char* who, hipStream_t stream) {
  BLVM_TRY(pchain_prepare(bld, who));
  const int rc = forward ? vrnn_static_fwd(bld.p, stream) : vrnn_static_bwd(bld.p, stream);
  return rc == 1 ? pchain_run(bld.p, stream) : rc;
}

}

extern "C" int blvm_pchain_static(int mode) {
  if (mode == -2) return (int)std::min<long>(blvm::g_static_launches, 0x7fffffffL);
  const int was = blvm::g_static;
  if (mode >= 0) blvm::g_static = mode != 0;
  return was;
}

static int static_chain_probe(const float* W16, const float* bias, float* x16, float* xs, int B, int N, int L, int nwg, void* stream_, bool resident) {
  using namespace blvm;
  using namespace blvm::pchain;
  hipStream_t s = static_cast<hipStream_t>(stream_);
  BLVM_REQUIRE(W16 && bias && x16 && xs && B > 0 && N > 0 && N % 16 == 0 && L > 0, "pchain_static_chain_probe: bad arguments");
  const int rt = (B + 15) / 16;
  const long x = (long)rt * 16 * N, sN = (long)B * N;
  Builder bld;
  bld.begin(OP_F32, L, B, 1, false, 0);
  const int nw = nwg > 0 ? nwg : range_for((N / 16) * rt, device_cus() & ~7);
  Operands o;
  o.p[LIN_A] = {x16, x}; o.p[LIN_W] = W16; o.p[LIN_BIAS] = bias; o.p[LIN_ORM] = {xs, sN}; o.p[LIN_O16] = {x16 + x, x}; o.ld[LD_OUT] = N; o.n16[N16_OUT] = N / 16;
  add_desc(bld, K_LIN, N / 16, 0, nw, N, DF_RELU, 0, L, o);
  BLVM_HIP(pchain_fill_sentinel(x16 + x, sizeof(float) * (size_t)x * L, s));
  BLVM_TRY(pchain_prepare(bld, "pchain_static_chain_probe"));
  const int rc = static_lin_chain_launch(bld.p, s, resident);
  BLVM_REQUIRE(rc != 1, "pchain_static_chain_probe: no static kernel for N = %d (256, 512) or this deal", N);
  return rc;
}
extern "C" int blvm_pchain_static_chain_probe(const float* W16, const float* bias, float* x16, float* xs, int B, int N, int L, int nwg, void* stream) {
  return static_chain_probe(W16, bias, x16, xs, B, N, L, nwg, stream, true);
}
extern "C" int blvm_pchain_static_chain_probe_fetch(const float* W16, const float* bias, float* x16, float* xs, int B, int N, int L, int nwg, void* stream) {
  return static_chain_probe(W16, bias, x16, xs, B, N, L, nwg, stream, false);
}
```

Before: 80.26 million.

## Defer epilogue argument setup to epilogue wave and write x16 before row-major

Turns the GRU, head, dz and GRU-backward tile routines into late variants. Epilogue pointer and argument structs are built lazily, and only by the first wave, inside the poll/prefetch window, so they are off the critical path. In the epilogue variants the polled x16 tile output is stored before the row-major copy, so downstream consumers see data sooner. The KL/dz terms are precomputed during the GEMM wait, and the head samples z before computing the remaining statistics. It also adds compile-time-gated timing instrumentation, and the dz maths is reordered with explicit FMAs, which may change rounding slightly.

```diff
diff --git a/benchmarking-lvms_amd/csrc/pchain.h b/benchmarking-lvms_amd/csrc/pchain.h
--- a/benchmarking-lvms_amd/csrc/pchain.h
+++ b/benchmarking-lvms_amd/csrc/pchain.h
@@ -70,11 +70,26 @@
   unsigned long long t_first = 0, t_ok = 0, t_end = 0, tp[8] = {0, 0, 0, 0, 0, 0, 0, 0};
   unsigned polls = 0;
 #endif
+#ifdef VRNN_STATIC_TPROF
+  unsigned long long vs[5] = {0, 0, 0, 0, 0}, vs_end = 0;
+  unsigned vs_polls = 0;
+  unsigned long long* vs_rec = nullptr;
+#endif
   __device__ __forceinline__ void sleep() const {
     if (nap > 8) __builtin_amdgcn_s_sleep(32);
     else __builtin_amdgcn_s_sleep(1);
   }
 };
+
+#ifdef VRNN_STATIC_TPROF
+#define VS_BEGIN(pl) do { const unsigned long long vs_t = wall_clock64(); for (int vs_i = 0; vs_i < 5; ++vs_i) (pl).vs[vs_i] = vs_t; (pl).vs_polls = 0; } while (0)
+#define VS_STAMP(pl, k) do { const unsigned long long vs_t = wall_clock64(); for (int vs_i = (k); vs_i < 5; ++vs_i) (pl).vs[vs_i] = vs_t; } while (0)
+#define VS_POLL(pl, first) do { if (first) VS_STAMP(pl, 1); ++(pl).vs_polls; } while (0)
+#else
+#define VS_BEGIN(pl) ((void)0)
+#define VS_STAMP(pl, k) ((void)0)
+#define VS_POLL(pl, first) ((void)0)
+#endif
 
 struct MapSame { static constexpr int of(int) { return 0; } static constexpr bool sum = false; };
 struct MapId { static constexpr int of(int g) { return g; } static constexpr bool sum = false; };
@@ -329,6 +344,7 @@
     for (int u = 0; u < NCH; ++u)
 #pragma unroll
       for (int g = 0; g < GA; ++g) a[g][u] = ld_sc1_x4(ar[g], aoff + 1024u * (unsigned)(u * NW));
+    VS_POLL(pl, mid_pending);
     if (mid_pending) { mid(); mid_pending = false; }
     bool bad = false;
 #pragma unroll
@@ -340,6 +356,7 @@
     pl.sleep();
   }
 multiply:
+  VS_STAMP(pl, 2);
   if constexpr (AMap::sum) {
 #pragma unroll
     for (int u = 0; u < NCH; ++u)
@@ -393,15 +410,23 @@
 };
 __device__ __forceinline__ Out out_rm(float* p, int ld, bool sc1 = false) { return Out{p, ld, sc1, nullptr, 0}; }
 __device__ __forceinline__ Out out_both(float* p, int ld, float* x16, int n16, bool sc1 = false) { return Out{p, ld, sc1, x16, n16}; }
-__device__ __forceinline__ void put(const Out& o, int r0, int c0, int row, int col, float x) {
+__device__ __forceinline__ void put_rm(const Out& o, int row, int col, float x) {
   if (o.rm != nullptr) {
     if (o.rm_sc1) st_sc1(make_rsrc(o.rm), 4u * ((unsigned)row * (unsigned)o.ld + (unsigned)col), x);
     else o.rm[(size_t)row * o.ld + col] = x;
   }
+}
+__device__ __forceinline__ void put_x16(const Out& o, int r0, int c0, int row, int col, float x) {
   const int rr = row - r0, cc = col - c0;
   const unsigned in_block = (unsigned)((rr + 16 * ((cc & 15) >> 2)) * 4 + (cc & 3));
   if (o.x16 != nullptr) st_sc1(make_rsrc(o.x16), 4u * ((((unsigned)(r0 >> 4) * (unsigned)o.n16 + (unsigned)((c0 + cc) >> 4)) << 8) + in_block), x);
   if (o.x16b != nullptr) st_sc1(make_rsrc(o.x16b), 4u * ((((unsigned)(r0 >> 4) * (unsigned)o.n16b + (unsigned)((c0 + cc) >> 4)) << 8) + in_block), x);
+}
+template <bool X16_FIRST = false>
+__device__ __forceinline__ void put(const Out& o, int r0, int c0, int row, int col, float x) {
+  if constexpr (!X16_FIRST) put_rm(o, row, col, x);
+  put_x16(o, r0, c0, row, col, x);
+  if constexpr (X16_FIRST) put_rm(o, row, col, x);
 }
 
 
@@ -446,6 +471,7 @@
   }
   float v[1];
   reduce_tiles<1, NW>(acc, red, v);
+  VS_STAMP(pl, 3);
 #ifdef PCHAIN_TPROF
   if (a_polled && pl.nap == 1) {
     const unsigned long long t3 = wall_clock64();
@@ -466,6 +492,7 @@
   if (L.relu) x = x > 0.f ? x : x * L.slope;
   if (L.gate) x = e_gate > 0.f ? x : x * L.slope;
   put(L.out, r0, c0, row, col, x);
+  VS_STAMP(pl, 4);
 #ifdef PCHAIN_TPROF
   if (a_polled && pl.nap == 1) { pl.t_end = wall_clock64(); }
 #endif
@@ -482,16 +509,28 @@
   float *mu_p, *sd_p, *mu_q, *sd_q, *raw_p, *raw_q, *muq_raw;
   Out z;
 };
-template <int NW, int OT = OP_F32, class WS = WMem>
-__device__ __forceinline__ void tile_head(const float* P, const float* Q, bool polled, const float* Wp, const float* bp, const float* Wq,
-                                          const float* bq, const float* eps, const HeadOut& o, int H, int Z, int residual, float beta,
-                                          float inv_beta, float sd_eps, int r0, int c0, int B, float* red, Poll& pl, const WS& ws = WS()) {
+__device__ __forceinline__ bool epilogue_wave() { return __builtin_amdgcn_readfirstlane((int)threadIdx.x) < 256; }
+
+struct HeadLate {
+  const float *bp, *bq, *eps;
+  HeadOut o;
+  int residual;
+  float beta, inv_beta, sd_eps;
+};
+template <int NW, int OT, bool EPI, class Late, class WS = WMem>
+__device__ __forceinline__ void tile_head_late(const float* P, const float* Q, bool polled, const float* Wp, const float* Wq, int H, int Z, Late& late,
+                                               int r0, int c0, int B, float* red, Poll& pl, const WS& ws = WS()) {
   const int t = threadIdx.x & 255;
   const int row = r0 + (t >> 4), col = c0 + (t & 15);
   const bool own = threadIdx.x < 256 && row < B;
   const size_t oc = (size_t)(row < B ? row : r0) * Z + col;
   float b0 = 0.f, b1 = 0.f, b2 = 0.f, b3 = 0.f, e = 0.f;
-  auto prefetch = [&]() { b0 = bp[col]; b1 = bp[Z + col]; b2 = bq[col]; b3 = bq[Z + col]; e = eps[oc]; };
+  HeadLate L;
+  auto prefetch = [&]() {
+    if (EPI && !epilogue_wave()) return;
+    L = late();
+    b0 = L.bp[col]; b1 = L.bp[Z + col]; b2 = L.bq[col]; b3 = L.bq[Z + col]; e = L.eps[oc];
+  };
   f32x4 acc[4];
 #pragma unroll
   for (int g = 0; g < 4; ++g) acc[g] = (f32x4){0.f, 0.f, 0.f, 0.f};
@@ -503,46 +542,76 @@
   }
   float v[4];
   reduce_tiles<4, NW>(acc, red, v);
+  VS_STAMP(pl, 3);
   if (!own) return;
+  const HeadOut& o = L.o;
   const size_t oo = (size_t)row * Z + col;
-  const float mp = v[0] + b0, rp = v[1] + b1, rq = v[3] + b3;
-  float mq = v[2] + b2;
-  const float sp = softplus_beta(rp, beta, inv_beta) + sd_eps;
-  const float sq = softplus_beta(rq, beta, inv_beta) + sd_eps;
-  if (o.muq_raw != nullptr) o.muq_raw[oo] = mq;
-  float sqc = sq;
-  if (residual == 1) {
-    mq += mp;
-  } else if (residual == 2) {
-    const float pq = 1.f / (sq * sq), pp = 1.f / (sp * sp);
-    const float var = 1.f / (pq + pp);
-    mq = var * (mq * pq + mp * pp);
-    sqc = sqrtf(var);
-  } else if (residual == 3) {
-    mq = mp;
-    sqc = sp;
-  }
-  put(o.z, r0, c0, row, col, e * sqc + mq);
+  const float mp = v[0] + b0, rp = v[1] + b1, rq = v[3] + b3, mq_raw = v[2] + b2;
+  auto sd = [&](float raw) { return softplus_beta(raw, L.beta, L.inv_beta) + L.sd_eps; };
+  auto sample = [&](float mu, float s) { put<EPI>(o.z, r0, c0, row, col, e * s + mu); VS_STAMP(pl, 4); };
+  float mq = mq_raw, sp, sqc;
+  if (EPI && L.residual < 2) {
+    sqc = sd(rq);
+    if (L.residual == 1) mq += mp;
+    sample(mq, sqc);
+    sp = sd(rp);
+  } else {
+    sp = sd(rp);
+    const float sq = sd(rq);
+    if (!EPI && o.muq_raw != nullptr) o.muq_raw[oo] = mq_raw;
+    sqc = sq;
+    if (L.residual == 1) {
+      mq += mp;
+    } else if (L.residual == 2) {
+      const float pq = 1.f / (sq * sq), pp = 1.f / (sp * sp);
+      const float var = 1.f / (pq + pp);
+      mq = var * (mq * pq + mp * pp);
+      sqc = sqrtf(var);
+    } else if (L.residual == 3) {
+      mq = mp;
+      sqc = sp;
+    }
+    sample(mq, sqc);
+  }
+  if (EPI && o.muq_raw != nullptr) o.muq_raw[oo] = mq_raw;
   o.mu_p[oo] = mp; o.sd_p[oo] = sp; o.mu_q[oo] = mq; o.sd_q[oo] = sqc;
   o.raw_p[oo] = rp; o.raw_q[oo] = rq;
 }
-
 template <int NW, int OT = OP_F32, class WS = WMem>
-__device__ __forceinline__ void tile_gru(const float* X, int ldx, bool polled, const float* Wih, int K, const float* xg, const float* bih,
-                                         const float* gh, const float* hprev, int ldh, int R, const Out& hnew, float* rg, float* ug, float* ng,
-                                         int r0, int c0, int B, float* red, Poll& pl, const WS& ws = WS()) {
+__device__ __forceinline__ void tile_head(const float* P, const float* Q, bool polled, const float* Wp, const float* bp, const float* Wq,
+                                          const float* bq, const float* eps, const HeadOut& o, int H, int Z, int residual, float beta,
+                                          float inv_beta, float sd_eps, int r0, int c0, int B, float* red, Poll& pl, const WS& ws = WS()) {
+  auto late = [&]() { return HeadLate{bp, bq, eps, o, residual, beta, inv_beta, sd_eps}; };
+  tile_head_late<NW, OT, false>(P, Q, polled, Wp, Wq, H, Z, late, r0, c0, B, red, pl, ws);
+}
+
+struct GruLate {
+  const float *xg, *bih, *gh, *hprev;
+  int ldh;
+  Out hnew;
+  float *rg, *ug, *ng;
+};
+template <int NW, int OT, bool EPI, class Late, class WS = WMem>
+__device__ __forceinline__ void tile_gru_late(const float* X, int ldx, bool polled, const float* Wih, int K, int R, Late& late, int r0, int c0, int B,
+                                              float* red, Poll& pl, const WS& ws = WS()) {
   const int t = threadIdx.x & 255;
   const int row = r0 + (t >> 4), col = c0 + (t & 15);
   const bool own = threadIdx.x < 256 && row < B;
   const int rowc = row < B ? row : r0;
   const size_t o3 = (size_t)rowc * 3 * R + col;
-  const rsrc_t rgh = make_rsrc(gh), rhp = make_rsrc(hprev);
-  const rsrc_t ps[4] = {rgh, rgh, rgh, rhp};
-  const unsigned po[4] = {4u * (unsigned)o3, 4u * (unsigned)(o3 + R), 4u * (unsigned)(o3 + 2 * R), 4u * ((unsigned)rowc * (unsigned)ldh + (unsigned)col)};
+  GruLate L;
+  rsrc_t ps[4];
+  unsigned po[4] = {4u * (unsigned)o3, 4u * (unsigned)(o3 + R), 4u * (unsigned)(o3 + 2 * R), 0u};
   float w[4] = {0.f, 0.f, 0.f, 0.f}, x0 = 0.f, x1 = 0.f, x2 = 0.f;
   auto prefetch = [&]() {
+    if (EPI && !epilogue_wave()) return;
+    L = late();
+    const rsrc_t rgh = make_rsrc(L.gh), rhp = make_rsrc(L.hprev);
+    ps[0] = rgh; ps[1] = rgh; ps[2] = rgh; ps[3] = rhp;
+    po[3] = 4u * ((unsigned)rowc * (unsigned)L.ldh + (unsigned)col);
 #pragma unroll
     for (int i = 0; i < 4; ++i) w[i] = ld_sc1(ps[i], po[i]);
+    const float *xg = L.xg, *bih = L.bih;
     x0 = (xg ? xg[o3] : 0.f) + (bih ? bih[col] : 0.f);
     x1 = (xg ? xg[o3 + R] : 0.f) + (bih ? bih[R + col] : 0.f);
     x2 = (xg ? xg[o3 + 2 * R] : 0.f) + (bih ? bih[2 * R + col] : 0.f);
@@ -558,15 +627,24 @@
   }
   float v[3];
   reduce_tiles<3, NW>(acc, red, v);
+  VS_STAMP(pl, 3);
   if (threadIdx.x >= 256) return;
   if (__any(own && (is_sentinel(w[0]) | is_sentinel(w[1]) | is_sentinel(w[2]) | is_sentinel(w[3])))) poll_words<4>(ps, po, w, own, pl);
   if (!own) return;
   const float r = sigmoidf_(v[0] + x0 + w[0]);
   const float u = sigmoidf_(v[1] + x1 + w[1]);
   const float n = tanhf(v[2] + x2 + r * w[2]);
-  put(hnew, r0, c0, row, col, (1.f - u) * n + u * w[3]);
+  put<EPI>(L.hnew, r0, c0, row, col, (1.f - u) * n + u * w[3]);
+  VS_STAMP(pl, 4);
   const size_t o = (size_t)row * R + col;
-  rg[o] = r; ug[o] = u; ng[o] = n;
+  L.rg[o] = r; L.ug[o] = u; L.ng[o] = n;
+}
+template <int NW, int OT = OP_F32, class WS = WMem>
+__device__ __forceinline__ void tile_gru(const float* X, int ldx, bool polled, const float* Wih, int K, const float* xg, const float* bih,
+                                         const float* gh, const float* hprev, int ldh, int R, const Out& hnew, float* rg, float* ug, float* ng,
+                                         int r0, int c0, int B, float* red, Poll& pl, const WS& ws = WS()) {
+  auto late = [&]() { return GruLate{xg, bih, gh, hprev, ldh, hnew, rg, ug, ng}; };
+  tile_gru_late<NW, OT, false>(X, ldx, polled, Wih, K, R, late, r0, c0, B, red, pl, ws);
 }
 
 struct DzIn {
@@ -577,27 +655,72 @@
   float fn_floor, beta, sd_eps;
   bool has_gemm = true;
 };
-template <int NW, int OT = OP_F32, class WS = WMem>
-__device__ __forceinline__ void tile_dz(const float* D, const float* WT, const float* D2, const float* WT2, bool polled, const float* dz_add,
-                                        int ld_add, bool add_polled, const DzIn& a, const Out& dqh, const Out& dph, int H, int Z, int r0, int c0,
-                                        int B, float* red, Poll& pl, const WS& ws = WS()) {
+struct DzTerms {
+  float ip2, t_muq, t_sdq, g_mup, g_sdp, sig_q, sig_p;
+};
+__device__ __forceinline__ DzTerms dz_terms(float mq, float sq, float mp, float sp, float rq, float rp, float c_raw, float c_fn, float fn_floor,
+                                            float beta) {
+#pragma clang fp contract(off)
+  DzTerms m;
+  const float d = mq - mp, ip2 = 1.f / (sp * sp);
+  const float ss = sq * sq + d * d;
+  float coef = c_raw;
+  if (c_fn != 0.f) {
+    const float k = __builtin_fmaf(ss * 0.5f, ip2, logf(sp) - logf(sq)) - 0.5f;
+    if (!(fn_floor > 0.f) || k > fn_floor) coef += c_fn;
+  }
+  m.ip2 = ip2;
+  m.t_muq = coef * d;
+  m.t_sdq = coef * __builtin_fmaf(sq, ip2, -(1.f / sq));
+  m.g_mup = -coef * d * ip2;
+  m.g_sdp = coef * (1.f / sp - ss * ip2 / sp);
+  m.sig_q = sigmoidf_(beta * rq);
+  m.sig_p = sigmoidf_(beta * rp);
+  return m;
+}
+struct DzLate {
+  const float* dz_add;
+  int ld_add;
+  bool add_polled;
+  DzIn a;
+  Out dqh, dph;
+};
+template <int NW, int OT, bool EPI, class Late, class WS = WMem>
+__device__ __forceinline__ void tile_dz_late(const float* D, const float* WT, const float* D2, const float* WT2, bool polled, bool has_gemm, Late& late,
+                                             int H, int Z, int r0, int c0, int B, float* red, Poll& pl, const WS& ws = WS()) {
   const int t = threadIdx.x & 255;
   const int row = r0 + (t >> 4), col = c0 + (t & 15);
   const bool own = threadIdx.x < 256 && row < B;
   const int rowc = row < B ? row : r0;
   const size_t o = (size_t)rowc * Z + col;
   float mq = 0.f, sq = 1.f, mp = 0.f, sp = 1.f, e = 0.f, rq = 0.f, rp = 0.f, c_raw = 0.f, c_fn = 0.f, e_add = 0.f;
-  auto prefetch = [&]() {
+  int x_len = 0;
+  DzLate L;
+  DzTerms m;
+  auto request = [&]() {
+    L = late();
+    const DzIn& a = L.a;
     mq = a.mu_q[o]; sq = a.sd_q[o]; mp = a.mu_p[o]; sp = a.sd_p[o]; e = a.eps[o]; rq = a.raw_q[o]; rp = a.raw_p[o];
     if (a.c_fn != nullptr || a.c_raw != nullptr) {
-      const bool live = (long long)a.t * a.stride < a.x_sl[rowc];
-      c_raw = (live && a.c_raw != nullptr) ? a.c_raw[rowc] : 0.f;
-      c_fn = (live && a.c_fn != nullptr) ? a.c_fn[rowc] : 0.f;
-    }
-    if (dz_add != nullptr && !add_polled) e_add = dz_add[(size_t)rowc * ld_add + col];
+      x_len = a.x_sl[rowc];
+      if (a.c_raw != nullptr) c_raw = a.c_raw[rowc];
+      if (a.c_fn != nullptr) c_fn = a.c_fn[rowc];
+    }
+    if (L.dz_add != nullptr && !L.add_polled) e_add = L.dz_add[(size_t)rowc * L.ld_add + col];
+  };
+  auto terms = [&]() {
+    const DzIn& a = L.a;
+    const bool live = (long long)a.t * a.stride < x_len;
+    m = dz_terms(mq, sq, mp, sp, rq, rp, live ? c_raw : 0.f, live ? c_fn : 0.f, a.fn_floor, a.beta);
+  };
+  const bool epi = EPI && epilogue_wave();
+  if (epi) request();
+  auto prefetch = [&]() {
+    if constexpr (!EPI) request();
+    else if (epi) terms();
   };
   float v[2] = {0.f, 0.f};
-  if (a.has_gemm) {
+  if (has_gemm) {
     f32x4 acc[2];
     acc[0] = (f32x4){0.f, 0.f, 0.f, 0.f};
     acc[1] = (f32x4){0.f, 0.f, 0.f, 0.f};
@@ -622,26 +745,25 @@
   } else {
     prefetch();
   }
+  VS_STAMP(pl, 3);
   if (threadIdx.x >= 256) return;
-  if (dz_add != nullptr && add_polled) {
-    const rsrc_t rs[1] = {make_rsrc(dz_add)};
-    const unsigned os[1] = {4u * ((unsigned)rowc * (unsigned)ld_add + (unsigned)col)};
+  const DzIn& a = L.a;
+  const Out &dqh = L.dqh, &dph = L.dph;
+  if (L.dz_add != nullptr && L.add_polled) {
+    const rsrc_t rs[1] = {make_rsrc(L.dz_add)};
+    const unsigned os[1] = {4u * ((unsigned)rowc * (unsigned)L.ld_add + (unsigned)col)};
     float ws[1];
     poll_words<1>(rs, os, ws, own, pl);
     e_add = ws[0];
   }
   if (!own) return;
+  if constexpr (!EPI) terms();
   const float dz = v[0] + v[1] + e_add;
-  const float d = mq - mp, ip2 = 1.f / (sp * sp);
-  float coef = c_raw;
-  if (c_fn != 0.f) {
-    const float k = logf(sp) - logf(sq) + (sq * sq + d * d) * 0.5f * ip2 - 0.5f;
-    if (!(a.fn_floor > 0.f) || k > a.fn_floor) coef += c_fn;
-  }
-  float g_muq = dz + coef * d * ip2;
-  float g_sdq = dz * e + coef * (sq * ip2 - 1.f / sq);
-  float g_mup = -coef * d * ip2;
-  float g_sdp = coef * (1.f / sp - (sq * sq + d * d) * ip2 / sp);
+  const float ip2 = m.ip2;
+  float g_muq = __builtin_fmaf(m.t_muq, ip2, dz);
+  float g_sdq = __builtin_fmaf(dz, e, m.t_sdq);
+  float g_mup = m.g_mup;
+  float g_sdp = m.g_sdp;
   if (a.residual == 1) {
     g_mup += g_muq;
   } else if (a.residual == 2) {
@@ -656,10 +778,18 @@
     g_sdq = g_pq * (-2.f * pq / sqr);
     g_muq = g_muq * var * pq;
   }
-  put(dqh, r0, c0, row, col, g_muq);
-  put(dqh, r0, Z + c0, row, Z + col, g_sdq * sigmoidf_(a.beta * rq));
-  put(dph, r0, c0, row, col, g_mup);
-  put(dph, r0, Z + c0, row, Z + col, g_sdp * sigmoidf_(a.beta * rp));
+  put<EPI>(dqh, r0, c0, row, col, g_muq);
+  VS_STAMP(pl, 4);
+  put<EPI>(dqh, r0, Z + c0, row, Z + col, g_sdq * m.sig_q);
+  put<EPI>(dph, r0, c0, row, col, g_mup);
+  put<EPI>(dph, r0, Z + c0, row, Z + col, g_sdp * m.sig_p);
+}
+template <int NW, int OT = OP_F32, class WS = WMem>
+__device__ __forceinline__ void tile_dz(const float* D, const float* WT, const float* D2, const float* WT2, bool polled, const float* dz_add,
+                                        int ld_add, bool add_polled, const DzIn& a, const Out& dqh, const Out& dph, int H, int Z, int r0, int c0,
+                                        int B, float* red, Poll& pl, const WS& ws = WS()) {
+  auto late = [&]() { return DzLate{dz_add, ld_add, add_polled, a, dqh, dph}; };
+  tile_dz_late<NW, OT, false>(D, WT, D2, WT2, polled, a.has_gemm, late, H, Z, r0, c0, B, red, pl, ws);
 }
 
 struct GrubIn {
@@ -670,15 +800,19 @@
   float *ga, *g_out;
   bool has_gemm, has_gin, has_gates;
 };
-template <int NW, int OT = OP_F32, class WS = WMem>
-__device__ __forceinline__ void tile_grub(const GrubIn& a, int K, int R, int r0, int c0, int B, float* red, Poll& pl, const WS& ws = WS()) {
+template <int NW, int OT, bool EPI, class Late, class WS = WMem>
+__device__ __forceinline__ void tile_grub_late(const float* D0, const float* D1, const float* W0, const float* W1, bool has_gemm, Late& late, int K, int R,
+                                               int r0, int c0, int B, float* red, Poll& pl, const WS& ws = WS()) {
   const int tt = threadIdx.x & 255;
   const int row = r0 + (tt >> 4), col = c0 + (tt & 15);
   const bool own = threadIdx.x < 256 && row < B;
   const int rowc = row < B ? row : r0;
   const size_t o = (size_t)rowc * R + col, o3 = (size_t)rowc * 3 * R + col;
   float r = 0.f, u = 0.f, n = 0.f, hn = 0.f, hp = 0.f, dd = 0.f, gadd = 0.f, g0 = 0.f;
+  GrubIn a;
   auto prefetch = [&]() {
+    if (EPI && !epilogue_wave()) return;
+    a = late();
     if (a.has_gin) g0 = ld_sc1(make_rsrc(a.g_in), 4u * (unsigned)o);
     if (a.has_gates) {
       r = a.rg[o]; u = a.ug[o]; n = a.ng[o]; hn = a.gh[o3 + 2 * R];
@@ -688,17 +822,18 @@
     if (a.g_add != nullptr) gadd = a.g_add[(size_t)rowc * a.ld_gadd + col];
   };
   float v[2] = {0.f, 0.f};
-  if (!a.has_gemm) prefetch();
-  if (a.has_gemm) {
+  if (!has_gemm) prefetch();
+  if (has_gemm) {
     f32x4 acc[2];
     acc[0] = (f32x4){0.f, 0.f, 0.f, 0.f};
     acc[1] = (f32x4){0.f, 0.f, 0.f, 0.f};
-    const float* const As[2] = {a.D0, a.D1};
-    const float* const Ws[2] = {a.W0, a.W1};
+    const float* const As[2] = {D0, D1};
+    const float* const Ws[2] = {W0, W1};
     const int la[2] = {0, 0}, cs[2] = {c0, c0};
     tile_product<NW, OT, 2, 2, MapId>(ws, As, la, true, r0, B, Ws, cs, K, acc, pl, prefetch);
     reduce_tiles<2, NW>(acc, red, v);
   }
+  VS_STAMP(pl, 3);
   if (threadIdx.x >= 256) return;
   if (a.has_gin && __any(own && is_sentinel(g0))) {
     const rsrc_t rs[1] = {make_rsrc(a.g_in)};
@@ -713,9 +848,23 @@
   const float dn_pre = g * (1.f - u) * (1.f - n * n);
   const float du_pre = g * (hp - n) * u * (1.f - u);
   const float dr_pre = dn_pre * hn * r * (1.f - r);
-  put(a.dgi, r0, c0, row, col, dr_pre); put(a.dgi, r0, R + c0, row, R + col, du_pre); put(a.dgi, r0, 2 * R + c0, row, 2 * R + col, dn_pre);
-  put(a.dgh, r0, c0, row, col, dr_pre); put(a.dgh, r0, R + c0, row, R + col, du_pre); put(a.dgh, r0, 2 * R + c0, row, 2 * R + col, dn_pre * r);
-  st_sc1(make_rsrc(a.ga), 4u * ((unsigned)row * (unsigned)R + (unsigned)col), g * u + dd);
+  const float ga = g * u + dd;
+  const unsigned oga = 4u * ((unsigned)row * (unsigned)R + (unsigned)col);
+  if constexpr (EPI) {
+    put_x16(a.dgi, r0, c0, row, col, dr_pre); VS_STAMP(pl, 4); put_x16(a.dgi, r0, R + c0, row, R + col, du_pre); put_x16(a.dgi, r0, 2 * R + c0, row, 2 * R + col, dn_pre);
+    st_sc1(make_rsrc(a.ga), oga, ga);
+    put<true>(a.dgh, r0, c0, row, col, dr_pre); put<true>(a.dgh, r0, R + c0, row, R + col, du_pre); put<true>(a.dgh, r0, 2 * R + c0, row, 2 * R + col, dn_pre * r);
+    put_rm(a.dgi, row, col, dr_pre); put_rm(a.dgi, row, R + col, du_pre); put_rm(a.dgi, row, 2 * R + col, dn_pre);
+  } else {
+    put(a.dgi, r0, c0, row, col, dr_pre); VS_STAMP(pl, 4); put(a.dgi, r0, R + c0, row, R + col, du_pre); put(a.dgi, r0, 2 * R + c0, row, 2 * R + col, dn_pre);
+    put(a.dgh, r0, c0, row, col, dr_pre); put(a.dgh, r0, R + c0, row, R + col, du_pre); put(a.dgh, r0, 2 * R + c0, row, 2 * R + col, dn_pre * r);
+    st_sc1(make_rsrc(a.ga), oga, ga);
+  }
+}
+template <int NW, int OT = OP_F32, class WS = WMem>
+__device__ __forceinline__ void tile_grub(const GrubIn& a, int K, int R, int r0, int c0, int B, float* red, Poll& pl, const WS& ws = WS()) {
+  auto late = [&]() { return a; };
+  tile_grub_late<NW, OT, false>(a.D0, a.D1, a.W0, a.W1, a.has_gemm, late, K, R, r0, c0, B, red, pl, ws);
 }
 
 __device__ __forceinline__ int seq_time_index(int j, int reverse, const int32_t* lens, int row) {
diff --git a/benchmarking-lvms_amd/csrc/vrnn_static.hip b/benchmarking-lvms_amd/csrc/vrnn_static.hip
--- a/benchmarking-lvms_amd/csrc/vrnn_static.hip
+++ b/benchmarking-lvms_amd/csrc/vrnn_static.hip
@@ -119,6 +119,36 @@
   }
 };
 
+#ifdef VRNN_STATIC_TPROF
+constexpr int kVsSlots = 40, kVsWords = 2 * 2 * kVsSlots * 8;
+constexpr unsigned long long kVsMagic = 0x7673616e61746f6dull;
+struct VsArgs {
+  unsigned long long* rec;
+  int wg[2];
+};
+__device__ __forceinline__ void vs_attach(Walk& wk, const VsArgs& v) {
+  const int w = blockIdx.x;
+  if (v.rec != nullptr && (w == v.wg[0] || w == v.wg[1])) wk.pl.vs_rec = v.rec + (w == v.wg[1] ? 2 * kVsSlots * 8 : 0);
+}
+__device__ __forceinline__ void vs_commit(Poll& pl, int slot) {
+  const unsigned long long t = wall_clock64();
+  const int wave = threadIdx.x >> 6;
+  if (pl.vs_rec != nullptr && (wave == 0 || wave == 4) && (threadIdx.x & 63) == 0) {
+    unsigned long long* r = pl.vs_rec + ((wave >> 2) * kVsSlots + slot) * 8;
+    r[0] += 1;
+    for (int k = 0; k < 4; ++k) r[1 + k] += pl.vs[k + 1] - pl.vs[k];
+    r[5] += t - pl.vs[4]; r[6] += pl.vs_polls;
+    if (pl.vs_end != 0) r[7] += pl.vs[0] - pl.vs_end;
+  }
+  pl.vs_end = t;
+}
+#define VS_COMMIT(pl, slot) vs_commit(pl, slot)
+#define VS_ARGS VsArgs vs;
+#else
+#define VS_COMMIT(pl, slot) ((void)0)
+#define VS_ARGS
+#endif
+
 template <int K, int G = 1>
 using Res = WRegs<OP_F32, G, K / 256>;
 template <int N, int K0, int K>
@@ -180,8 +210,10 @@
   };
   for (int tk = 0; tk < (WS::resident ? 1 : nt); ++tk) {
     const int trc = __builtin_amdgcn_readlane(tiles, tk), tr0 = trc & 0xffff, tc0 = (trc >> 16) * 16;
+    VS_BEGIN(wk.pl);
     if constexpr ((FLAGS & DF_CANARY) != 0) canary_wait(A, tr0, K, wk.pl, q.ld0);
     tile_lin_late<NW, OP_F32>(A, q.ld0, true, q.W, K, late, tr0, tc0, wk.B, wk.red(), wk.pl, A2, A3, q.w_width, ws);
+    VS_COMMIT(wk.pl, 4 * d.idx);
   }
 }
 
@@ -193,6 +225,7 @@
 #pragma unroll
   for (int li = 0; li < N; ++li) {
     wk.at(d, s, false, (unsigned)li);
+    VS_BEGIN(wk.pl);
     auto late = [&]() {
       const float* aux = q.aux[li].at(s);
       return LinLate{GATED ? nullptr : aux, li == 0 ? q.add0.at(s) : nullptr, GATED ? aux : nullptr, q.ldadd0, q.ldgate, false, !GATED, q.slope,
@@ -200,6 +233,7 @@
     };
     if (li == 0) tile_lin_late<NW, OP_F32>(A, 0, true, q.W[li], K0, late, tr0, tc0, wk.B, wk.red(), wk.pl, nullptr, nullptr, 0, rr.first);
     else tile_lin_late<NW, OP_F32>(A, 0, true, q.W[li], K, late, tr0, tc0, wk.B, wk.red(), wk.pl, nullptr, nullptr, 0, rr.rest[li > 0 ? li - 1 : 0]);
+    VS_COMMIT(wk.pl, 4 * d.idx + li);
     A = q.o16[li].at(s);
   }
 }
@@ -208,53 +242,76 @@
 __device__ __forceinline__ void visit_head(const HeadArgs& q, const Deal& d, int s, int tiles, int nt, Walk& wk, const Res<kH, 4>& ws) {
   if (nt == 0 || s < d.s_begin || s >= d.s_end) return;
   wk.at(d, s, false);
-  const HeadOut o{q.mu_p.at(s), q.sd_p.at(s), q.mu_q.at(s), q.sd_q.at(s), q.raw_p.at(s), q.raw_q.at(s), q.muq_raw.at(s),
-                  Out{q.z.at(s), q.ld3, false, q.z16.at(s), q.n16, q.z16b.at(s), q.n16b}};
+  VS_BEGIN(wk.pl);
+  auto late = [&]() {
+    return HeadLate{q.bp, q.bq, q.eps.at(s),
+                    HeadOut{q.mu_p.at(s), q.sd_p.at(s), q.mu_q.at(s), q.sd_q.at(s), q.raw_p.at(s), q.raw_q.at(s), q.muq_raw.at(s),
+                            Out{q.z.at(s), q.ld3, false, q.z16.at(s), q.n16, q.z16b.at(s), q.n16b}},
+                    q.residual, q.beta, q.inv_beta, q.sd_eps};
+  };
   const int trc = __builtin_amdgcn_readlane(tiles, 0);
-  tile_head<NW, OP_F32>(q.P.at(s), q.Q.at(s), true, q.Wp, q.bp, q.Wq, q.bq, q.eps.at(s), o, kH, q.Z, q.residual, q.beta, q.inv_beta, q.sd_eps,
-                        trc & 0xffff, (trc >> 16) * 16, wk.B, wk.red(), wk.pl, ws);
+  tile_head_late<NW, OP_F32, true>(q.P.at(s), q.Q.at(s), true, q.Wp, q.Wq, kH, q.Z, late, trc & 0xffff, (trc >> 16) * 16, wk.B, wk.red(), wk.pl, ws);
+  VS_COMMIT(wk.pl, 4 * d.idx);
 }
 
 template <int NW>
 __device__ __forceinline__ void visit_gru(const GruArgs& q, const Deal& d, int s, int tiles, int nt, Walk& wk, const Res<kH, 3>& ws) {
   if (nt == 0 || s < d.s_begin || s >= d.s_end) return;
   wk.at(d, s, false);
-  const Out o{q.hrm.at(s), q.ld3, true, q.h16.at(s), q.n16, q.h16b.at(s), q.n16b};
+  VS_BEGIN(wk.pl);
+  auto late = [&]() {
+    return GruLate{q.xg.at(s), q.bih, q.gh.at(s), q.hprev.at(s), q.ld0, Out{q.hrm.at(s), q.ld3, true, q.h16.at(s), q.n16, q.h16b.at(s), q.n16b},
+                   q.rg.at(s), q.ug.at(s), q.ng.at(s)};
+  };
   const int trc = __builtin_amdgcn_readlane(tiles, 0);
-  tile_gru<NW, OP_F32>(q.X.at(s), 0, true, q.Wih, kH, q.xg.at(s), q.bih, q.gh.at(s), q.hprev.at(s), q.ld0, q.R, o, q.rg.at(s), q.ug.at(s), q.ng.at(s),
-                       trc & 0xffff, (trc >> 16) * 16, wk.B, wk.red(), wk.pl, ws);
+  tile_gru_late<NW, OP_F32, true>(q.X.at(s), 0, true, q.Wih, kH, q.R, late, trc & 0xffff, (trc >> 16) * 16, wk.B, wk.red(), wk.pl, ws);
+  VS_COMMIT(wk.pl, 4 * d.idx);
 }
 
 template <int NW>
 __device__ __forceinline__ void visit_dz(const DzArgs& q, const Deal& d, int s, int tiles, int nt, Walk& wk, const Res<kH>& ws) {
   if (nt == 0 || s < d.s_begin || s >= d.s_end) return;
   wk.at(d, s, false);
-  DzIn z;
-  z.mu_q = q.mu_q.at(s); z.sd_q = q.sd_q.at(s); z.mu_p = q.mu_p.at(s); z.sd_p = q.sd_p.at(s); z.eps = q.eps.at(s); z.raw_q = q.raw_q.at(s);
-  z.raw_p = q.raw_p.at(s); z.muq_raw = q.muq_raw.at(s);
-  z.x_sl = q.x_sl; z.c_raw = q.c_raw; z.c_fn = q.c_fn;
-  z.t = q.t0 - s; z.stride = q.stride; z.residual = q.residual;
-  z.fn_floor = q.fn_floor; z.beta = q.beta; z.sd_eps = q.sd_eps;
-  z.has_gemm = s >= q.first_gemm;
-  const Out oq{q.dqh.at(s), q.ld3, false, q.dqh16.at(s), q.n16}, op{q.dph.at(s), q.ld3, false, q.dph16.at(s), q.n16};
+  VS_BEGIN(wk.pl);
+  auto late = [&]() {
+    DzLate l;
+    l.dz_add = q.add.at(s); l.ld_add = q.ld1; l.add_polled = false;
+    DzIn& z = l.a;
+    z.mu_q = q.mu_q.at(s); z.sd_q = q.sd_q.at(s); z.mu_p = q.mu_p.at(s); z.sd_p = q.sd_p.at(s); z.eps = q.eps.at(s); z.raw_q = q.raw_q.at(s);
+    z.raw_p = q.raw_p.at(s); z.muq_raw = q.muq_raw.at(s);
+    z.x_sl = q.x_sl; z.c_raw = q.c_raw; z.c_fn = q.c_fn;
+    z.t = q.t0 - s; z.stride = q.stride; z.residual = q.residual;
+    z.fn_floor = q.fn_floor; z.beta = q.beta; z.sd_eps = q.sd_eps;
+    l.dqh = Out{q.dqh.at(s), q.ld3, false, q.dqh16.at(s), q.n16};
+    l.dph = Out{q.dph.at(s), q.ld3, false, q.dph16.at(s), q.n16};
+    return l;
+  };
   const int trc = __builtin_amdgcn_readlane(tiles, 0);
-  tile_dz<NW, OP_F32>(q.D.at(s), q.WT, nullptr, nullptr, true, q.add.at(s), q.ld1, false, z, oq, op, kH, q.Z, trc & 0xffff, (trc >> 16) * 16, wk.B,
-                      wk.red(), wk.pl, ws);
+  tile_dz_late<NW, OP_F32, true>(q.D.at(s), q.WT, nullptr, nullptr, true, s >= q.first_gemm, late, kH, q.Z, trc & 0xffff, (trc >> 16) * 16, wk.B, wk.red(),
+                                 wk.pl, ws);
+  VS_COMMIT(wk.pl, 4 * d.idx);
 }
 
 template <int NW>
 __device__ __forceinline__ void visit_grub(const GrubArgs& q, const Deal& d, int s, int tiles, int nt, Walk& wk, const Res<kH, 2>& ws) {
   if (nt == 0 || s < d.s_begin || s >= d.s_end) return;
   wk.at(d, s, false);
-  GrubIn g;
-  g.D0 = q.D0.at(s); g.D1 = q.D1.at(s); g.W0 = q.W0; g.W1 = q.W1; g.g_in = q.g_in.at(s); g.g_add = q.g_add.at(s); g.ld_gadd = q.ld1;
-  g.rg = q.rg.at(s); g.ug = q.ug.at(s); g.ng = q.ng.at(s); g.gh = q.gh.at(s); g.hprev = q.hprev.at(s); g.dd = q.dd.at(s); g.ldh = q.ld0;
-  g.dgi = Out{q.dgi.at(s), q.ld3, false, q.dgi16.at(s), q.n16};
-  g.dgh = Out{q.dgh.at(s), q.ld3, false, q.dgh16.at(s), q.n16};
-  g.ga = q.ga.at(s); g.g_out = const_cast<float*>(q.g_out);
-  g.has_gemm = s >= q.first_gemm; g.has_gates = s < q.end_gates; g.has_gin = s >= q.first_gin;
+  VS_BEGIN(wk.pl);
+  auto late = [&]() {
+    GrubIn g;
+    g.D0 = nullptr; g.D1 = nullptr; g.W0 = nullptr; g.W1 = nullptr;
+    g.g_in = q.g_in.at(s); g.g_add = q.g_add.at(s); g.ld_gadd = q.ld1;
+    g.rg = q.rg.at(s); g.ug = q.ug.at(s); g.ng = q.ng.at(s); g.gh = q.gh.at(s); g.hprev = q.hprev.at(s); g.dd = q.dd.at(s); g.ldh = q.ld0;
+    g.dgi = Out{q.dgi.at(s), q.ld3, false, q.dgi16.at(s), q.n16};
+    g.dgh = Out{q.dgh.at(s), q.ld3, false, q.dgh16.at(s), q.n16};
+    g.ga = q.ga.at(s); g.g_out = const_cast<float*>(q.g_out);
+    g.has_gemm = s >= q.first_gemm; g.has_gates = s < q.end_gates; g.has_gin = s >= q.first_gin;
+    return g;
+  };
   const int trc = __builtin_amdgcn_readlane(tiles, 0);
-  tile_grub<NW, OP_F32>(g, kH, q.R, trc & 0xffff, (trc >> 16) * 16, wk.B, wk.red(), wk.pl, ws);
+  tile_grub_late<NW, OP_F32, true>(q.D0.at(s), q.D1.at(s), q.W0, q.W1, s >= q.first_gemm, late, kH, q.R, trc & 0xffff, (trc >> 16) * 16, wk.B, wk.red(),
+                                   wk.pl, ws);
+  VS_COMMIT(wk.pl, 4 * d.idx);
 }
 
 template <class A>
@@ -274,6 +331,7 @@
   Deal deal[6];
   int B, s0, S, xcd;
   Ctl ctl;
+  VS_ARGS
 };
 constexpr int kFwdProducts = 4, kBwdProducts = 2;
 
@@ -305,6 +363,9 @@
   const int w = blockIdx.x, rt = (a.B + 15) / 16;
   const bool xcd = a.xcd != 0;
   Walk wk{lds_red, lds_red + kFwdProducts * NW * 256, 0, a.B, Poll{a.ctl, 0u, false, 1}};
+#ifdef VRNN_STATIC_TPROF
+  vs_attach(wk, a.vs);
+#endif
   if (w >= a.deal[0].wg0) {
     const int t0 = tile_lanes(w, a.deal[0].wg0, a.deal[0].nwg, rt, a.deal[0].ct, xcd), n0 = tile_count(t0);
     if (n0 == 0) return;
@@ -324,6 +385,7 @@
   Deal deal[10];
   int B, s0, S, xcd;
   Ctl ctl;
+  VS_ARGS
 };
 
 template <int NW, int HALF>
@@ -361,6 +423,9 @@
   const int w = blockIdx.x, rt = (a.B + 15) / 16;
   const bool xcd = a.xcd != 0;
   Walk wk{lds_red, lds_red + kBwdProducts * NW * 256, 0, a.B, Poll{a.ctl, 0u, false, 1}};
+#ifdef VRNN_STATIC_TPROF
+  vs_attach(wk, a.vs);
+#endif
   if (w >= a.deal[3].wg0) {
     const int t = tile_lanes(w, a.deal[3].wg0, a.deal[3].nwg, rt, a.deal[3].ct, xcd), n = tile_count(t);
     if (n == 0) return;
@@ -456,6 +521,28 @@
   q.ldadd0 = d.i[LINSEQ_I_LD_ADD0]; q.ldgate = d.i[LINSEQ_I_LD_GATE]; q.n16 = d.n16[N16_OUT]; q.slope = d.f[LINSEQ_F_SLOPE];
   return q;
 }
+
+#ifdef VRNN_STATIC_TPROF
+VsArgs vs_args(const Program& p, bool backward, int half_wg0, int end_wg, const int (&first)[2], int nfirst, const int* shared, int nshared) {
+  VsArgs v{nullptr, {-1, -1}};
+  unsigned long long* buf = pchain_profile_buffer();
+  unsigned long long magic = 0;
+  if (buf == nullptr || hipMemcpy(&magic, buf, sizeof(magic), hipMemcpyDeviceToHost) != hipSuccess || magic != kVsMagic) return v;
+  v.rec = buf + 1 + (backward ? kVsWords : 0);
+  const int rt = (p.B + 15) / 16;
+  for (int h = 0; h < 2; ++h) {
+    int best = -1;
+    for (int w = h == 0 ? 0 : half_wg0; w < (h == 0 ? half_wg0 : end_wg); ++w) {
+      int n = 0;
+      auto has = [&](const Desc& d) { return TileIter(w, d.wg0, d.nwg, rt, d.ct, p.xcd != 0).valid() ? 1 : 0; };
+      for (int k = 0; k < nfirst; ++k) n += has(p.d[first[h] + (k > 0 ? 7 * k : 0)]);
+      for (int k = 0; k < nshared; ++k) n += has(p.d[shared[k]]);
+      if (n > best) { best = n; v.wg[h] = w; }
+    }
+  }
+  return v;
+}
+#endif
 
 int vrnn_static_check(const Program& p, int ndesc, int products) {
   if (!pchain_static_on() || p.ndesc != ndesc || p.ot != OP_F32 || p.rt_group != 1 || p.s_first != 0 || p.B > 64) return 1;
@@ -494,6 +581,12 @@
   int grid = 0;
   for (int i = 0; i < 6; ++i) { a.deal[i] = deal_of(d[i], i); grid = std::max(grid, d[i].wg0 + d[i].nwg); }
   a.B = p.B; a.s0 = p.s_first; a.S = S; a.xcd = p.xcd; a.ctl = p.ctl;
+#ifdef VRNN_STATIC_TPROF
+  {
+    const int first[2] = {1, 2}, shared[3] = {3, 4, 5};
+    a.vs = vs_args(p, false, half, gentle, first, 1, shared, 3);
+  }
+#endif
   const size_t lds = sizeof(float) * 2 * kFwdProducts * 16 * 256;
   BLVM_TRY(static_go(&vrnn_static_fwd_kernel<16>, 0, grid, lds, "vrnn_static_fwd"));
   hipLaunchKernelGGL(vrnn_static_fwd_kernel<16>, dim3(grid), dim3(1024), lds, stream, a);
@@ -539,6 +632,12 @@
   int grid = 0;
   for (int i = 0; i < 10; ++i) { a.deal[i] = deal_of(d[i], i); grid = std::max(grid, d[i].wg0 + d[i].nwg); }
   a.B = p.B; a.s0 = p.s_first; a.S = S; a.xcd = p.xcd; a.ctl = p.ctl;
+#ifdef VRNN_STATIC_TPROF
+  {
+    const int first[2] = {1, 2}, shared[4] = {0, 5, 6, 7};
+    a.vs = vs_args(p, true, half, gentle, first, 2, shared, 4);
+  }
+#endif
   const size_t lds = sizeof(float) * 2 * kBwdProducts * 16 * 256;
   BLVM_TRY(static_go(&vrnn_static_bwd_kernel<16>, 1, grid, lds, "vrnn_static_bwd"));
   hipLaunchKernelGGL(vrnn_static_bwd_kernel<16>, dim3(grid), dim3(1024), lds, stream, a);
```

Result: no change. 80.95 million, median of 6 (+0.9%).
